# plainerman/DiffDock-Pocket

Measured on AMD Instinct MI355X. Metric: ligand poses/sec (40 samples x 20 steps) on 3dpf, higher is better.
Workload: dtype f32 (fc and G products: fp16 hi/lo split of both operands on v_mfma_f32_16x16x32_f16 - the row-stationary conv kernel - and v_mfma_f32_32x32x16_f16, fp32 accumulate; G between its two kernels as fp16 hi + continuation byte = 19 significant bits; the exact fp32 MFMA form is timed in other_workloads)

## Files before the change

diffdock_pocket_amd/_lib.py:

```python
from __future__ import annotations

import ctypes as C
import operator
import os

HERE = os.path.dirname(os.path.abspath(__file__))
LIB_PATH = os.environ.get("DDP_HIP_LIB", os.path.join(HERE, "libddp_hip.so"))

DDP_MAX_TASKS, DDP_MAX_BLOCKS, DDP_MAX_SEGS, DDP_MAX_NS, DDP_EDGE_TILE = 9, 4, 3, 64, 64
F_SCALAR_S0, F_DOT, F_SCALAR_S1, F_VEC_S0, F_CROSS = range(5)
FS = 68

DDP_MAX_GEMM_BATCH = 16
DDP_EVAL_MAX_ATOMS = 1024
DDP_GUIDANCE_MAX_TORSIONS = 1024
DDP_MINIMIZE_MAX_ATOMS, DDP_MINIMIZE_MAX_TORSIONS = 512, 4096
DDP_MINIMIZE_FLEX_MAX_MOVING, DDP_MINIMIZE_FLEX_MAX_BONDS, DDP_MINIMIZE_FLEX_MAX_STATE_BYTES = 256, 256, 47040
DDP_SCORE_GUIDANCE_FLEX_MAX_ATOMS, DDP_SCORE_GUIDANCE_FLEX_MAX_TORSIONS = DDP_MINIMIZE_MAX_ATOMS, DDP_GUIDANCE_MAX_TORSIONS
DDP_SCORE_GUIDANCE_FLEX_MAX_MOVING, DDP_SCORE_GUIDANCE_FLEX_MAX_BONDS = DDP_MINIMIZE_FLEX_MAX_MOVING, DDP_MINIMIZE_FLEX_MAX_BONDS
DDP_PAIRWISE_MAX_SAMPLES, DDP_CLUSTER_MAX_SAMPLES = 32768, 1024
EXPORTS = ["ddp_conv_messages", "ddp_conv_rows", "ddp_stage_a_gh", "ddp_stage_a_gh3", "ddp_segment_reduce", "ddp_edge_featurize", "ddp_edge_featurize_jobs", "ddp_torsion_sh", "ddp_stage_a", "ddp_stage_a_h2",
           "ddp_pose_update", "ddp_sidechain_update", "ddp_sde_update", "ddp_radius_count", "ddp_radius_fill", "ddp_knn", "ddp_group_by_key", "ddp_node_linear", "ddp_scan_jobs", "ddp_mark_jobs", "ddp_rowcopy_jobs", "ddp_select_jobs",
           "ddp_gather_rows", "ddp_clean_pair_maps", "ddp_flex_mark", "ddp_fallback_rowmap", "ddp_step_prologue", "ddp_trrot_head", "ddp_tor_head", "ddp_radius_search_jobs", "ddp_group_by_key_jobs", "ddp_set_occupancy_shaping", "ddp_pose_rmsd", "ddp_pose_contacts", "ddp_pose_pairwise_rmsd", "ddp_pose_cluster", "ddp_traj_record", "ddp_svgd_tau", "ddp_svgd_pairs", "ddp_svgd_rows", "ddp_refine_energy", "ddp_refine_direction", "ddp_refine_accept", "ddp_clash_guidance", "ddp_score_guidance", "ddp_score_guidance_flex", "ddp_pose_score", "ddp_pose_profile", "ddp_pose_minimize", "ddp_pose_minimize_flex", "ddp_pose_search", "ddp_pose_search_select", "ddp_pose_search_flex", "ddp_pocket_occupancy", "ddp_pocket_buriedness", "ddp_pocket_label", "ddp_conv_deal_tile", "ddp_abi_version", "ddp_last_error", "ddp_source_hash"]


class Seg(C.Structure):
    _fields_ = [("kind", C.c_int32), ("in_off", C.c_int32), ("count", C.c_int32)]


class Block(C.Structure):
    _fields_ = [("U", C.c_int32), ("n", C.c_int32), ("C", C.c_int32), ("out_off", C.c_int32), ("tile0", C.c_int32),
                ("ntiles", C.c_int32), ("nsub", C.c_int32), ("ups", C.c_int32), ("nseg", C.c_int32),
                ("seg", Seg * DDP_MAX_SEGS), ("g_slot", C.c_int32), ("g_col0", C.c_int32)]


class RoleSeg(C.Structure):
    _fields_ = [("block", C.c_int32), ("tile0", C.c_int32), ("tstride", C.c_int32), ("count", C.c_int32), ("round", C.c_int32)]


DDP_CONV32_WAVES, DDP_MAX_ROLE_SEGS = 4, 2


class ConvShape(C.Structure):
    _fields_ = [("f_in", C.c_int32), ("hid", C.c_int32), ("kp1", C.c_int32), ("hp", C.c_int32), ("hs", C.c_int32),
                ("nct1", C.c_int32), ("d_out", C.c_int32), ("nblocks", C.c_int32), ("fbuf_floats", C.c_int32),
                ("g_cols", C.c_int32 * 2), ("blk", Block * DDP_MAX_BLOCKS), ("nrounds", C.c_int32),
                ("nrole", C.c_int32 * DDP_CONV32_WAVES), ("role", (RoleSeg * DDP_MAX_ROLE_SEGS) * DDP_CONV32_WAVES)]


class ConvTask(C.Structure):
    _fields_ = [("x_src", C.c_void_p), ("ldx_src", C.c_int32), ("n_edges", C.c_int32), ("src", C.c_void_p),
                ("eid", C.c_void_p), ("sh", C.c_void_p), ("seg_ptr", C.c_void_p * DDP_MAX_SEGS),
                ("seg_idx", C.c_void_p * DDP_MAX_SEGS), ("seg_ld", C.c_int32 * DDP_MAX_SEGS),
                ("seg_n", C.c_int32 * DDP_MAX_SEGS), ("w1p", C.c_void_p), ("b1p", C.c_void_p), ("w2p", C.c_void_p),
                ("b2p", C.c_void_p), ("msg", C.c_void_p), ("g", C.c_void_p * 2),
                ("pos", C.c_void_p), ("n_edges_dev", C.c_void_p), ("w1h", C.c_void_p), ("w2h", C.c_void_p), ("h2_range_flag", C.c_void_p),
                ("wsh", C.c_void_p), ("bsp", C.c_void_p), ("gh", C.c_void_p * 2), ("gh_fmt", C.c_int32), ("rows_form", C.c_int32), ("rows_bias_k", C.c_int32), ("rows_seg0", C.c_int32), ("rows_seg1", C.c_int32), ("rows_nts", C.c_int32)]


class ReduceSrc(C.Structure):
    _fields_ = [("msg", C.c_void_p), ("rowptr", C.c_void_p), ("bn_scale", C.c_void_p), ("bn_shift", C.c_void_p),
                ("n_edges", C.c_int32), ("rowmap", C.c_void_p), ("n_edges_dev", C.c_void_p)]


DDP_MAX_NODE_JOBS, DDP_MAX_NODE_CAT = 8, 16
DDP_MAX_LIST_JOBS = 12
_P, _I = C.c_void_p, C.c_int32


class ScanJob(C.Structure):
    _fields_ = [("n", _I), ("n_dev", _P), ("flag", _P), ("val", _P), ("rowptr", _P), ("base", _I), ("excl", _P), ("excl2", _P),
                ("list", _P), ("total", _P)]


class MarkJob(C.Structure):
    _fields_ = [("idx", _P), ("n", _I), ("n_dev", _P), ("mask", _P)]


class RowcopyJob(C.Structure):
    _fields_ = [("n_rows", _I), ("keep", _P), ("old_rowptr", _P), ("new_rowptr", _P), ("inp", _P * 3), ("out", _P * 3)]


class SelectJob(C.Structure):
    _fields_ = [("n", _I), ("n_dev", _P), ("mask_a", _P), ("idx_a", _P), ("mask_b", _P), ("idx_b", _P), ("out_idx", _P),
                ("pay", _P * 4), ("pay_add", _I * 4), ("out", _P * 4), ("total", _P), ("block_count", _P), ("block_off", _P)]


class RadiusJob(C.Structure):
    _fields_ = [("x", _P), ("x_ptr", _P), ("y", _P), ("y_batch", _P), ("ny", _I), ("r", C.c_float), ("max_neighbors", _I),
                ("flags", _I), ("graph_div", _P), ("counts", _P), ("offsets", _P), ("base", _I), ("total", _P), ("out_query", _P),
                ("out_x", _P), ("capacity", _I), ("overflow", _P)]


class SdeArgs(C.Structure):
    _fields_ = [("score", _P * 4), ("z", _P * 4), ("out", _P * 4), ("n", _I * 4)]


class SvgdArgs(C.Structure):
    _fields_ = [("pos", _P), ("n", _I), ("n_lig", _I), ("n_tor", _I), ("dihedrals", _P), ("score", _P * 3), ("upd", _P * 3), ("gdt", _P),
                ("weight", C.c_float), ("w_rep", C.c_float), ("w_rot", C.c_float), ("w_tor", C.c_float), ("svgd_only", _I),
                ("tau", _P), ("tr_diff", _P), ("rot_diff", _P), ("tor_diff", _P), ("dist", _P)]


class RefineArgs(C.Structure):
    _fields_ = [("n_samples", _I), ("n", _I), ("m", _I), ("rec_stride", _I), ("n_tor", _I), ("pos", _P), ("anchor", _P), ("lig_radii", _P),
                ("rec", _P), ("rec_radii", _P), ("self_pairs", _P), ("overlap", C.c_double), ("restraint", C.c_double), ("energy", _P),
                ("grad", _P), ("bonds", _P), ("mask_rotate", _P), ("step", _P), ("tr", _P), ("rot", _P), ("tor", _P), ("trial", _P),
                ("trial_energy", _P), ("trial_grad", _P), ("accepted", _P), ("grow", C.c_double), ("shrink", C.c_double),
                ("step_max", C.c_double)]


class GuidanceArgs(C.Structure):
    _fields_ = [("n_samples", _I), ("n", _I), ("m", _I), ("rec_stride", _I), ("n_tor", _I), ("pos", _P), ("lig_radii", _P), ("rec", _P),
                ("rec_radii", _P), ("self_pairs", _P), ("bonds", _P), ("mask_rotate", _P), ("overlap", C.c_double), ("weight", _P),
                ("max_tr", C.c_double), ("max_rot", C.c_double), ("max_tor", C.c_double), ("upd", _P * 3), ("energy", _P), ("grad", _P)]


class ScoreForm(C.Structure):
    _fields_ = [(k, C.c_double) for k in ("cutoff", "gauss_offset", "gauss_width", "hydrophobic_good", "hydrophobic_bad", "hbond_good",
                                          "hbond_bad", "w_gauss", "w_repulsion", "w_hydrophobic", "w_hbond")]
    _read = operator.attrgetter(*(k for k, _ in _fields_))

    @classmethod
    def from_config(cls, config) -> "ScoreForm":
        return cls(*cls._read(config))


class ScoreArgs(C.Structure):
    _anonymous_ = ("form",)
    _fields_ = [("n_samples", _I), ("n", _I), ("m", _I), ("rec_stride", _I), ("pos", _P), ("lig_radii", _P), ("lig_flags", _P), ("rec", _P),
                ("rec_radii", _P), ("rec_flags", _P), ("self_pairs", _P), ("form", ScoreForm), ("tor_divisor", C.c_double), ("energy", _P),
                ("grad", _P)]


class ScoreGuidanceArgs(C.Structure):
    _anonymous_ = ("form",)
    _fields_ = [("n_samples", _I), ("n", _I), ("m", _I), ("rec_stride", _I), ("n_tor", _I), ("pos", _P), ("lig_radii", _P), ("lig_flags", _P),
                ("rec", _P), ("rec_radii", _P), ("rec_flags", _P), ("self_pairs", _P), ("bonds", _P), ("mask_rotate", _P), ("form", ScoreForm),
                ("weight", _P), ("max_tr", C.c_double), ("max_rot", C.c_double), ("max_tor", C.c_double), ("upd", _P * 3), ("energy", _P),
                ("grad", _P)]


class ScoreGuidanceFlexArgs(C.Structure):
    _anonymous_ = ("form",)
    _fields_ = ScoreGuidanceArgs._fields_[:-2] + [("n_mov", _I), ("n_sc", _I), ("n_sub", _I), ("reserved", _I), ("mov", _P), ("sc_edge_idx", _P),
                                                  ("sc_sub", _P), ("sc_map", _P), ("sc_pairs", _P), ("max_sc", C.c_double), ("upd_sc", _P),
                                                  ("energy", _P), ("grad_mov", _P)]


class ProfileArgs(C.Structure):
    _anonymous_ = ("form",)
    _fields_ = [("n_samples", _I), ("n", _I), ("m", _I), ("rec_stride", _I), ("n_res", _I), ("reserved", _I), ("pos", _P), ("lig_radii", _P),
                ("lig_flags", _P), ("rec", _P), ("rec_radii", _P), ("rec_flags", _P), ("res_ptr", _P), ("form", ScoreForm),
                ("contact_distance", C.c_double), ("profile", _P), ("bits", _P)]


class MinimizeArgs(C.Structure):
    _anonymous_ = ("form",)
    _fields_ = [("n_samples", _I), ("n", _I), ("m", _I), ("rec_stride", _I), ("n_tor", _I), ("iterations", _I), ("pos", _P), ("anchor", _P),
                ("lig_radii", _P), ("lig_flags", _P), ("rec", _P), ("rec_radii", _P), ("rec_flags", _P), ("self_pairs", _P), ("bonds", _P),
                ("mask_rotate", _P), ("form", ScoreForm), ("restraint", C.c_double), ("grow", C.c_double), ("shrink", C.c_double),
                ("step_max", C.c_double), ("step", _P), ("accepted", _P), ("energy_in", _P), ("energy_out", _P), ("history", _P), ("grad", _P)]


class MinimizeFlexArgs(C.Structure):
    _anonymous_ = ("form",)
    _fields_ = MinimizeArgs._fields_ + [("rec_anchor", _P), ("n_mov", _I), ("n_sc", _I), ("n_sub", _I), ("reserved", _I), ("mov", _P),
                                        ("sc_edge_idx", _P), ("sc_sub", _P), ("sc_map", _P), ("sc_pairs", _P),
                                        ("restraint_sc", C.c_double), ("grad_mov", _P)]


class SearchArgs(C.Structure):
    _fields_ = [("min", MinimizeArgs), ("replicas", _I), ("cycles", _I), ("cycle0", _I), ("reserved", _I), ("step_init", C.c_double),
                ("temperature", C.c_double), ("perturb", _P), ("u", _P), ("cur_pos", _P), ("cur_e", _P), ("best_pos", _P), ("best_e", _P),
                ("best_cycle", _P), ("accepted", _P), ("trace", _P), ("flags", _P), ("starts", _P)]


class SearchFlexArgs(C.Structure):
    _fields_ = [("flex", MinimizeFlexArgs), ("replicas", _I), ("cycles", _I), ("cycle0", _I), ("reserved", _I), ("step_init", C.c_double),
                ("temperature", C.c_double), ("perturb", _P), ("u", _P), ("cur_pos", _P), ("cur_mov", _P), ("cur_e", _P), ("best_pos", _P),
                ("best_mov", _P), ("best_e", _P), ("best_cycle", _P), ("accepted", _P), ("trace", _P), ("flags", _P), ("starts", _P),
                ("starts_mov", _P)]


class SearchSelectArgs(C.Structure):
    _fields_ = [("n_samples", _I), ("n", _I), ("replicas", _I), ("reserved", _I), ("best_pos", _P), ("best_e", _P), ("best_cycle", _P),
                ("pos_out", _P), ("energy_out", _P), ("replica_out", _P), ("cycle_out", _P)]


def flex_state_bytes(n: int, n_mov: int, n_sc: int) -> int:
    return 89 * n + 81 * n_mov + 4 * n_sc


class GroupJob(C.Structure):
    _fields_ = [("key", _P), ("n_items", _I), ("n_items_dev", _P), ("n_keys", _I), ("pay", _P * 3), ("rowptr", _P), ("perm", _P),
                ("out_key", _P), ("out", _P * 3), ("key_map", _P), ("scratch", _P)]



DDP_MAX_FEATURIZE_JOBS = 8


class FeaturizeJob(C.Structure):
    _fields_ = [("pos_a", _P), ("ia", _P), ("pos_b", _P), ("ib", _P), ("n_edges", _I), ("n_edges_dev", _P), ("offset", _P), ("k_rbf", _I),
                ("coeff", C.c_float), ("pre", _P), ("pre_idx", _P), ("ld_pre", _I), ("pre2", _P), ("n_pre2", _I), ("ld_pre2", _I),
                ("w1d", _P), ("w2", _P), ("b2", _P), ("ns", _I), ("out", _P), ("sh", _P)]


class _BondJob(C.Structure):
    _fields_ = [("pos", _P), ("b0", _P), ("b1", _P), ("n", _I), ("mid", _P), ("vec", _P)]


class _CopyJob(C.Structure):
    _fields_ = [("src", _P), ("dst", _P), ("n", _I)]


class PrologueArgs(C.Structure):
    _fields_ = [("t", _P * 4), ("t_stride", _I * 4), ("sig_min", C.c_float * 4), ("sig_max", C.c_float * 4), ("sigma", _P * 4),
                ("n_graphs", _I), ("cut", _P), ("cut_mul", C.c_float), ("cut_add", C.c_float), ("graph_emb", _P), ("sd", _I),
                ("emb_scale", C.c_float), ("freq", _P), ("lig_pos", _P), ("graph_ptr", _P), ("center", _P),
                ("bonds", _BondJob * 2), ("copy", _CopyJob * 2)]


class TrRotArgs(C.Structure):
    _fields_ = [("gp", _P), ("ld_gp", _I), ("n_graphs", _I), ("ns", _I), ("sd", _I), ("graph_emb", _P), ("w1", _P * 2), ("b1", _P * 2),
                ("w2", _P * 2), ("b2", _P * 2), ("sigma", _P * 2), ("so3_table", _P), ("so3_n", _I), ("so3_lo", C.c_float),
                ("so3_span", C.c_float), ("out", _P * 2)]


class TorArgs(C.Structure):
    _fields_ = [("h", _P), ("ld_h", _I), ("n_bonds", _I), ("ns", _I), ("w1", _P), ("w2", _P), ("sigma", _P), ("graph_of_bond", _P),
                ("torus_table", _P), ("torus_n", _I), ("torus_lo", C.c_float), ("torus_span", C.c_float), ("out", _P)]


class NodeJob(C.Structure):
    _fields_ = [("n_rows", C.c_int32), ("cat", C.c_void_p), ("ld_cat", C.c_int32), ("n_cat", C.c_int32), ("table", C.c_void_p),
                ("feat_off", C.c_int32 * DDP_MAX_NODE_CAT), ("emb_dim", C.c_int32), ("emb_mode", C.c_int32),
                ("dense", C.c_void_p * 2), ("ld_dense", C.c_int32 * 2), ("n_dense", C.c_int32 * 2),
                ("t", C.c_void_p), ("t_stride", C.c_int32), ("scale", C.c_float), ("freq", C.c_void_p),
                ("sig_emb", C.c_void_p), ("ld_sig", C.c_int32), ("sd", C.c_int32), ("sig_out", C.c_void_p), ("ld_sig_out", C.c_int32),
                ("w", C.c_void_p), ("bias", C.c_void_p),
                ("out", C.c_void_p), ("ld_out", C.c_int32), ("ncols", C.c_int32), ("zero_to", C.c_int32),
                ("add", C.c_void_p), ("ld_add", C.c_int32)]


def g_ld(hid: int, gcols: int) -> int:
    return (((hid + 3) // 4 * 4 + 1) * gcols + 31) // 32 * 32


class DdpError(RuntimeError):
    pass


_lib = None


def load():
    global _lib
    if _lib is not None:
        return _lib
    if not os.path.exists(LIB_PATH):
        raise DdpError(f"{LIB_PATH} not found: build it with `python -m diffdock_pocket_amd.build` "
                       f"(hipcc --offload-arch=gfx950); there is no fallback path")
    lib = C.CDLL(LIB_PATH)
    for name in EXPORTS:
        if not hasattr(lib, name):
            raise DdpError(f"{LIB_PATH} does not export {name}")
    lib.ddp_abi_version.restype = C.c_int
    lib.ddp_last_error.restype = C.c_char_p
    lib.ddp_conv_messages.argtypes = [C.POINTER(ConvShape), C.POINTER(ConvTask), C.c_int, C.c_void_p]
    lib.ddp_conv_messages.restype = C.c_int
    lib.ddp_conv_rows.argtypes = lib.ddp_conv_messages.argtypes
    lib.ddp_conv_rows.restype = C.c_int
    lib.ddp_segment_reduce.argtypes = [C.c_void_p, C.c_int, C.c_int, C.c_int, C.POINTER(ReduceSrc), C.c_int, C.c_int,
                                       C.c_int, C.c_int, C.c_void_p]
    lib.ddp_segment_reduce.restype = C.c_int
    lib.ddp_edge_featurize.argtypes = [C.c_void_p, C.c_void_p, C.c_void_p, C.c_void_p, C.c_int, C.c_void_p, C.c_void_p, C.c_int,
                                       C.c_float, C.c_void_p, C.c_void_p, C.c_int, C.c_void_p, C.c_int, C.c_int, C.c_void_p,
                                       C.c_void_p, C.c_void_p, C.c_int, C.c_void_p, C.c_void_p, C.c_void_p]
    lib.ddp_edge_featurize.restype = C.c_int
    lib.ddp_edge_featurize_jobs.argtypes = [C.POINTER(FeaturizeJob), C.c_int, C.c_void_p]
    lib.ddp_edge_featurize_jobs.restype = C.c_int
    lib.ddp_torsion_sh.argtypes = [C.c_void_p, C.c_void_p, C.c_void_p, C.c_int, C.c_void_p, C.c_void_p, C.c_void_p, C.c_int, C.c_int,
                                   C.c_void_p, C.c_void_p, C.c_int, C.c_void_p, C.c_void_p]
    lib.ddp_torsion_sh.restype = C.c_int
    lib.ddp_stage_a.argtypes = [C.c_void_p, C.c_int, C.c_int, C.c_void_p, C.c_void_p, C.c_int, C.POINTER(C.c_int32), C.c_int,
                                C.c_void_p, C.c_void_p, C.c_int, C.c_int, C.c_void_p, C.c_int, C.c_void_p]
    lib.ddp_stage_a.restype = C.c_int
    lib.ddp_stage_a_h2.argtypes = lib.ddp_stage_a.argtypes[:-1] + [C.c_void_p, C.c_void_p]
    lib.ddp_stage_a_h2.restype = C.c_int
    lib.ddp_stage_a_gh.argtypes = lib.ddp_stage_a_h2.argtypes[:-1] + [C.c_void_p, C.c_void_p]
    lib.ddp_stage_a_gh.restype = C.c_int
    lib.ddp_stage_a_gh3.argtypes = lib.ddp_stage_a_gh.argtypes
    lib.ddp_stage_a_gh3.restype = C.c_int
    lib.ddp_set_occupancy_shaping.argtypes = [C.c_int, C.c_int]
    lib.ddp_set_occupancy_shaping.restype = C.c_int
    lib.ddp_pose_update.argtypes = [C.c_void_p, C.c_int, C.c_int, C.c_void_p, C.c_void_p, C.c_void_p, C.c_int, C.c_void_p,
                                    C.c_void_p, C.c_void_p, C.c_void_p]
    lib.ddp_pose_update.restype = C.c_int
    lib.ddp_sidechain_update.argtypes = [C.c_void_p, C.c_int, C.c_int, C.c_void_p, C.c_int, C.c_void_p, C.c_void_p, C.c_void_p,
                                         C.c_void_p, C.c_void_p]
    lib.ddp_sidechain_update.restype = C.c_int
    lib.ddp_radius_count.argtypes = [C.c_void_p, C.c_void_p, C.c_void_p, C.c_void_p, C.c_int, C.c_float, C.c_int, C.c_int,
                                     C.c_void_p, C.c_void_p]
    lib.ddp_radius_count.restype = C.c_int
    lib.ddp_radius_fill.argtypes = [C.c_void_p, C.c_void_p, C.c_void_p, C.c_void_p, C.c_int, C.c_float, C.c_int, C.c_int,
                                    C.c_void_p, C.c_void_p, C.c_void_p, C.c_void_p]
    lib.ddp_radius_fill.restype = C.c_int
    lib.ddp_knn.argtypes = [C.c_void_p, C.c_void_p, C.c_void_p, C.c_int, C.c_int, C.c_void_p, C.c_void_p]
    lib.ddp_knn.restype = C.c_int
    lib.ddp_group_by_key.argtypes = [C.c_void_p, C.c_int, C.c_int] + [C.c_void_p] * 11
    lib.ddp_group_by_key.restype = C.c_int
    for name, job in (("ddp_scan_jobs", ScanJob), ("ddp_mark_jobs", MarkJob), ("ddp_rowcopy_jobs", RowcopyJob),
                      ("ddp_select_jobs", SelectJob), ("ddp_radius_search_jobs", RadiusJob), ("ddp_group_by_key_jobs", GroupJob)):
        getattr(lib, name).argtypes = [C.POINTER(job), C.c_int, C.c_void_p]
        getattr(lib, name).restype = C.c_int
    lib.ddp_sde_update.argtypes = [C.c_void_p, C.POINTER(SdeArgs), C.c_void_p]
    lib.ddp_sde_update.restype = C.c_int
    lib.ddp_gather_rows.argtypes = [C.c_void_p, C.c_int, C.c_void_p, C.c_int, C.c_void_p, C.c_void_p, C.c_int, C.c_int, C.c_void_p]
    lib.ddp_gather_rows.restype = C.c_int
    lib.ddp_clean_pair_maps.argtypes = [C.c_void_p, C.c_void_p, C.c_void_p, C.c_void_p, C.c_int, C.c_int, C.c_int, C.c_int, C.c_void_p,
                                        C.c_void_p, C.c_void_p]
    lib.ddp_clean_pair_maps.restype = C.c_int
    lib.ddp_flex_mark.argtypes = [C.c_void_p, C.c_void_p, C.c_int, C.c_void_p, C.c_void_p, C.c_int, C.c_int, C.c_int, C.c_int, C.c_int,
                                  C.c_void_p, C.c_void_p]
    lib.ddp_flex_mark.restype = C.c_int
    lib.ddp_fallback_rowmap.argtypes = [C.c_void_p, C.c_void_p, C.c_void_p, C.c_void_p, C.c_int, C.c_int, C.c_void_p, C.c_void_p]
    lib.ddp_fallback_rowmap.restype = C.c_int
    for name, st in (("ddp_step_prologue", PrologueArgs), ("ddp_trrot_head", TrRotArgs), ("ddp_tor_head", TorArgs)):
        getattr(lib, name).argtypes = [C.POINTER(st), C.c_void_p]
        getattr(lib, name).restype = C.c_int
    lib.ddp_node_linear.argtypes = [C.POINTER(NodeJob), C.c_int, C.c_void_p]
    lib.ddp_node_linear.restype = C.c_int
    lib.ddp_pose_rmsd.argtypes = [C.c_void_p, C.c_int, C.c_int, C.c_void_p, C.c_int, C.c_void_p, C.c_int, C.c_void_p, C.c_int,
                                  C.c_void_p, C.c_void_p, C.c_void_p]
    lib.ddp_pose_rmsd.restype = C.c_int
    lib.ddp_pose_contacts.argtypes = [C.c_void_p, C.c_int, C.c_int, C.c_void_p, C.c_void_p, C.c_int, C.c_int, C.c_void_p, C.c_float,
                                      C.c_void_p, C.c_void_p, C.c_void_p]
    lib.ddp_pose_contacts.restype = C.c_int
    lib.ddp_pose_pairwise_rmsd.argtypes = [C.c_void_p, C.c_int, C.c_int, C.c_void_p, C.c_int, C.c_void_p, C.c_int, C.c_void_p, C.c_void_p]
    lib.ddp_pose_pairwise_rmsd.restype = C.c_int
    lib.ddp_pose_cluster.argtypes = [C.c_void_p, C.c_int, C.c_void_p, C.c_float, C.c_void_p, C.c_void_p, C.c_void_p, C.c_void_p, C.c_void_p]
    lib.ddp_pose_cluster.restype = C.c_int
    lib.ddp_traj_record.argtypes = [C.c_void_p, C.c_int, C.c_int, C.c_void_p, C.c_void_p, C.c_int, C.c_void_p, C.c_int, C.c_void_p,
                                    C.c_int, C.c_void_p, C.c_void_p]
    lib.ddp_traj_record.restype = C.c_int
    for name in ("ddp_svgd_tau", "ddp_svgd_pairs", "ddp_svgd_rows"):
        getattr(lib, name).argtypes = [C.POINTER(SvgdArgs), C.c_void_p]
        getattr(lib, name).restype = C.c_int
    for name in ("ddp_refine_energy", "ddp_refine_direction", "ddp_refine_accept"):
        getattr(lib, name).argtypes = [C.POINTER(RefineArgs), C.c_void_p]
        getattr(lib, name).restype = C.c_int
    lib.ddp_clash_guidance.argtypes = [C.POINTER(GuidanceArgs), C.c_void_p]
    lib.ddp_clash_guidance.restype = C.c_int
    lib.ddp_score_guidance.argtypes = [C.POINTER(ScoreGuidanceArgs), C.c_void_p]
    lib.ddp_score_guidance.restype = C.c_int
    lib.ddp_score_guidance_flex.argtypes = [C.POINTER(ScoreGuidanceFlexArgs), C.c_void_p]
    lib.ddp_score_guidance_flex.restype = C.c_int
    lib.ddp_pose_score.argtypes = [C.POINTER(ScoreArgs), C.c_void_p]
    lib.ddp_pose_score.restype = C.c_int
    lib.ddp_pose_profile.argtypes = [C.POINTER(ProfileArgs), C.c_void_p]
    lib.ddp_pose_profile.restype = C.c_int
    lib.ddp_pose_minimize.argtypes = [C.POINTER(MinimizeArgs), C.c_void_p]
    lib.ddp_pose_minimize.restype = C.c_int
    lib.ddp_pose_minimize_flex.argtypes = [C.POINTER(MinimizeFlexArgs), C.c_void_p]
    lib.ddp_pose_minimize_flex.restype = C.c_int
    lib.ddp_pose_search.argtypes = [C.POINTER(SearchArgs), C.c_void_p]
    lib.ddp_pose_search.restype = C.c_int
    lib.ddp_pose_search_select.argtypes = [C.POINTER(SearchSelectArgs), C.c_void_p]
    lib.ddp_pose_search_select.restype = C.c_int
    lib.ddp_pose_search_flex.argtypes = [C.POINTER(SearchFlexArgs), C.c_void_p]
    lib.ddp_pose_search_flex.restype = C.c_int
    lib.ddp_pocket_occupancy.argtypes = [C.c_void_p, C.c_void_p, C.c_int, C.c_float, C.c_float, C.c_float, C.c_float, C.c_int, C.c_int, C.c_int,
                                         C.c_void_p, C.c_void_p]
    lib.ddp_pocket_occupancy.restype = C.c_int
    lib.ddp_pocket_buriedness.argtypes = [C.c_void_p, C.c_int, C.c_int, C.c_int, C.c_double, C.c_double, C.c_int, C.c_void_p, C.c_void_p,
                                          C.c_void_p]
    lib.ddp_pocket_buriedness.restype = C.c_int
    lib.ddp_pocket_label.argtypes = [C.c_void_p, C.c_int, C.c_int, C.c_int, C.c_void_p, C.c_void_p]
    lib.ddp_pocket_label.restype = C.c_int
    lib.ddp_conv_deal_tile.argtypes = [C.c_int, C.c_int, C.c_int]
    lib.ddp_conv_deal_tile.restype = C.c_int
    if lib.ddp_abi_version() != 17:
        raise DdpError("libddp_hip.so ABI version mismatch")
    lib.ddp_source_hash.restype = C.c_char_p
    if "DDP_HIP_LIB" not in os.environ:
        from .build import source_hash
        have, want = lib.ddp_source_hash().decode(), source_hash()
        if have != want:
            raise DdpError(f"{LIB_PATH} was built from other sources (library {have}, tree {want}): rebuild it with "
                           f"`python -m diffdock_pocket_amd.build`")
    _lib = lib
    return lib


def check(rc, what):
    if rc != 0:
        raise DdpError(f"{what} failed (rc={rc}): {load().ddp_last_error().decode()}")
```

diffdock_pocket_amd/csrc/ddp_conv_rows.hip:

```cpp
#include <hip/hip_runtime.h>
#include <stdint.h>
#include <stdio.h>
#include <stdlib.h>

#undef DDP_STAMPS
#include "ddp_conv_rows_common.h"

#ifndef DDP_ROWS_GRING1
#define DDP_ROWS_GRING1 12
#endif
#ifndef DDP_ROWS_GRING3
#define DDP_ROWS_GRING3 8
#endif

#ifdef DDP_ROWS_STAMPS
#define RS_SLOTS 32
#define RS_WGS 16384
__device__ unsigned long long ddp_rows_stamp_buf[(size_t)RS_WGS * ROWS_NW * RS_SLOTS];
#define RSTAMP(k)                                                                                          \
  do {                                                                                                     \
    unsigned long long t_;                                                                                 \
    __builtin_amdgcn_sched_barrier(0);                                                                     \
    asm volatile("s_memtime %0\n\ts_waitcnt lgkmcnt(0)" : "=s"(t_)::"memory");                          \
    __builtin_amdgcn_sched_barrier(0);                                                                     \
// ... 486 lines not shown
  {
    int lo = 1 << 30, hi = 0;
    for (int bi = 0; bi < S.nblocks; ++bi)
      if (S.blk[bi].ntiles > 0)
        for (int si = 0; si < S.blk[bi].nseg; ++si) {
          lo = min(lo, S.blk[bi].seg[si].in_off);
          hi = max(hi, S.blk[bi].seg[si].in_off + 3 * S.blk[bi].seg[si].count);
        }
    const float* __restrict__ xs = T.x_src + (size_t)src * T.ldx_src;
#pragma unroll
    for (int i = 0; i < 2; ++i) vtouch[i] = (hi > lo) ? xs[min(lo + 32 * (2 * i + hh), hi - 1)] : 0.f;
  }

  rows_request_piece<NS>(ring, wsh, 0, ROWS_NP * RL.nts, 0, wave, lane);
  rows_request_piece<NS>(ring, wsh, 1, ROWS_NP * RL.nts, 1, wave, lane);
  for (int i = tid; i < RL.nts * 32; i += ROWS_NT) lbias[i] = T.bsp[i];
  RSTAMP(1);
  h8 xh[NS];
  f32x4* xlo = reinterpret_cast<f32x4*>(priv);
  {
    f32x4 xv[NS][2];
#pragma unroll
    for (int ks = 0; ks < NS; ++ks)
#pragma unroll
      for (int q = 0; q < 2; ++q) {
        const int kq = 4 * ks + 2 * hh + q;
        const int sg = kq / NQ, off = kq - sg * NQ;
        const float* __restrict__ b = (sg == 0) ? xb0 : (sg == 1) ? xb1 : xb2;
        xv[ks][q] = (sg < 3) ? reinterpret_cast<const f32x4*>(b)[off] : f32x4{0.f, 0.f, 0.f, 0.f};
      }
#pragma unroll
    for (int ks = 0; ks < NS; ++ks) {
      h4 h0, l0, h1, l1;
      rows_split(xv[ks][0], ROWS_SX, h0, l0, T.h2_range_flag);
      rows_split(xv[ks][1], ROWS_SX, h1, l1, T.h2_range_flag);
      h8 lo;
#pragma unroll
      for (int i = 0; i < 4; ++i) {
        xh[ks][i] = h0[i];
        xh[ks][4 + i] = h1[i];
        lo[i] = l0[i];
        lo[4 + i] = l1[i];
      }
      xlo[ks * 64 + lane] = __builtin_bit_cast(f32x4, lo);
    }
  }

  RSTAMP(2);
  asm volatile("" ::"v"(vtouch[0]), "v"(vtouch[1]));
  h8 ah[NS], al[NS];
  int t = 0;
#pragma unroll
  for (int ct = 0; ct < NCT1; ++ct, ++t) {
    f32x16 acc;
#pragma unroll
    for (int pc = 0; pc < ROWS_NP; ++pc) {
      constexpr int KPP = NS / ROWS_NP, PIECE_Q = 2 * KPP * 64;
      if (pc == 0) rows_stream_step<NS, 0>(ring, wsh, t, RL.nts, wave, lane);
      else if (pc == 1) rows_stream_step<NS, 1>(ring, wsh, t, RL.nts, wave, lane);
      else rows_stream_step<NS, 2>(ring, wsh, t, RL.nts, wave, lane);
      if (pc == 0) {
        const f32x4* bp = reinterpret_cast<const f32x4*>(lbias + t * 32 + 4 * hh);
#pragma unroll
        for (int q4 = 0; q4 < 4; ++q4) {
          const f32x4 b = bp[2 * q4];
#pragma unroll
          for (int q = 0; q < 4; ++q) acc[4 * q4 + q] = b[q];
        }
      }
      const f32x4* slot = ring + pc * PIECE_Q;
      f32x4 w0 = slot[lane], w1 = slot[64 + lane];
      f32x4 xl = xlo[(pc * KPP) * 64 + lane];
#pragma unroll
      for (int k = 0; k < KPP; ++k) {
        const int ks = pc * KPP + k;
        const h8 wh = __builtin_bit_cast(h8, w0), wl = __builtin_bit_cast(h8, w1), xlk = __builtin_bit_cast(h8, xl);
        if (k + 1 < KPP) {
          w0 = slot[(2 * k + 2) * 64 + lane];
          w1 = slot[(2 * k + 3) * 64 + lane];
          xl = xlo[(ks + 1) * 64 + lane];
        }
        acc = __builtin_amdgcn_mfma_f32_32x32x16_f16(wh, xh[ks], acc, 0, 0, 0);
        acc = __builtin_amdgcn_mfma_f32_32x32x16_f16(wh, xlk, acc, 0, 0, 0);
        acc = __builtin_amdgcn_mfma_f32_32x32x16_f16(wl, xh[ks], acc, 0, 0, 0);
      }
    }
#pragma unroll
    for (int j = 0; j < 16; ++j) {
      const float pre = acc[j] * (ROWS_SH / (ROWS_SW * ROWS_SX));
      h2_range_check(pre, T.h2_range_flag);
      const float v = fmaxf(pre, 0.f);
      const _Float16 hi = (_Float16)v;
      const _Float16 lo = (_Float16)(v - (float)hi);
      if (2 * ct + (j >> 3) < NS) {
        ah[2 * ct + (j >> 3)][j & 7] = hi;
        al[2 * ct + (j >> 3)][j & 7] = lo;
      }
    }
  }

  RSTAMP(3);
  float* F = reinterpret_cast<float*>(priv);
  RowsAux* aux = reinterpret_cast<RowsAux*>(priv + RL.aux_off);
  unsigned rmask;
  {
    const int prev = __shfl_up(src, 1);
    const bool rowv = (hh == 0) && (r < nvw);
    const bool runstart = rowv && (r == 0 || src != prev);
    rmask = (unsigned)(__ballot(runstart) & 0xffffffffull);
    const unsigned upto = (r == 31) ? ~0u : ((2u << r) - 1u);
    if (hh == 0) {
      aux->src[r] = src;
      aux->pos[r] = pos;
      aux->rid[r] = rowv ? (int)__popc(rmask & upto) - 1 : -1;
      constexpr float fs = 1.f / (ROWS_SH * ROWS_SW), gs = 1.f / (ROWS_SH * ROWS_SG);
      aux->sh[r][0] = shv[0] * fs; aux->sh[r][1] = shv[1] * fs; aux->sh[r][2] = shv[2] * fs; aux->sh[r][3] = shv[3] * fs;
      aux->shT[0][r] = shv[0] * gs; aux->shT[1][r] = shv[1] * gs; aux->shT[2][r] = shv[2] * gs; aux->shT[3][r] = shv[3] * gs;
    }
  }

  RSTAMP(4);
  RSTAMP_VAL(30, __popc(rmask));
  RSTAMP_VAL(31, p0 / ROWS_ET);
  int sgi = 0;
  for (int bi = 0; bi < S.nblocks; ++bi) {
    const ddp_block_t& B = S.blk[bi];
    if (B.ntiles > 0 && B.U > 0) {
      bool fast = true;
      for (int si = 0; si < B.nseg; ++si)
        fast = fast && B.seg[si].count <= 16 && (B.seg[si].kind == DDP_F_DOT || B.seg[si].kind == DDP_F_VEC_S0 || B.seg[si].kind == DDP_F_CROSS);
      if (fast)
        rows_build_features<8>(B, T, aux, F, lane);
      else
        build_features<32, 2>(B, T, aux->src, aux->sh, F, lane);
    }
    const int nparts = (B.n + 31) >> 5;
    for (int part = 0; part < nparts; ++part, ++sgi) {
      int gmode = 0;
      if (B.C == 3 && B.g_slot >= 0 && nparts == 1 && 2 * B.n <= 32) {
        const bool with_next = bi + 1 < S.nblocks && S.blk[bi + 1].C == 3 && S.blk[bi + 1].g_slot >= 0 && S.blk[bi + 1].n == B.n;
        const bool with_prev = bi > 0 && S.blk[bi - 1].C == 3 && S.blk[bi - 1].g_slot >= 0 && S.blk[bi - 1].n == B.n;
        const bool prev_is_second = with_prev && bi > 1 && S.blk[bi - 2].C == 3 && S.blk[bi - 2].g_slot >= 0 && S.blk[bi - 2].n == B.n;
        if (with_prev && !prev_is_second) gmode = 2;
        else if (with_next) gmode = 1;
      }
      if (B.C == 1)
        t = rows_segment<NS, 1, G3>(RL, B, bi, part, T, ah, al, ring, lbias, t, F, aux, rmask, src, nvw, wave, lane, sgi, 0);
      else
        t = rows_segment<NS, 3, G3>(RL, B, bi, part, T, ah, al, ring, lbias, t, F, aux, rmask, src, nvw, wave, lane, sgi, gmode);
    }
  }
}

int ddp_conv_rows_plan(const ddp_conv_shape_t* shape, const ddp_conv_task_t* tasks, int ntasks, RowsPlan* plan) {
  if (!shape || !tasks) return ddp_fail(DDP_EINVAL, "ddp_conv_rows: null argument");
  if (ntasks < 0 || ntasks > DDP_MAX_TASKS) return ddp_fail(DDP_ELIMIT, "ddp_conv_rows: ntasks > DDP_MAX_TASKS");
  if (shape->nblocks < 1 || shape->nblocks > DDP_MAX_BLOCKS) return ddp_fail(DDP_EINVAL, "ddp_conv_rows: nblocks");
  const int sc = (shape->f_in != shape->hid) ? 0 : (shape->hid == 180) ? 60 : (shape->hid == 96) ? 32 : 0;
  if (sc == 0) return ddp_fail(DDP_EINVAL, "ddp_conv_rows: shapes of the size classes ns = 60 / 32 (f_in = hid = 180 / 96) only");
  RowsPlan& P = *plan;
  ConvLaunch& L = P.L;
  L.shape = *shape;
  L.r1_floats = 0;
  L.tv_off = 0;
  L.ntasks = 0;
  L.dev_counts = 0;
  L.deal_c = ddp_conv_deal_chunk();
  const int NS = (sc == 60) ? 12 : 6, nct1 = shape->nct1;
  if (nct1 != (shape->hid + 31) / 32) return ddp_fail(DDP_EINVAL, "ddp_conv_rows: nct1");
  int nts = nct1, frows = 0;
  for (int b = 0; b < shape->nblocks; ++b) {
    const ddp_block_t& B = shape->blk[b];
    if (B.C != 1 && B.C != 3) return ddp_fail(DDP_EINVAL, "ddp_conv_rows: block C must be 1 or 3");
    if (B.n < 1 || B.n > 64 || (B.C == 3 && B.n > 32)) return ddp_fail(DDP_ELIMIT, "ddp_conv_rows: block n too large");
    if (B.nsub < 1 || B.nsub > 2 || B.ups < 1 || (B.nsub > 1) != (B.n > 32) || (B.nsub == 1 && B.ups != 32 / B.n))
      return ddp_fail(DDP_EINVAL, "ddp_conv_rows: nsub / ups");
    if (B.g_slot > 1 || (B.g_slot >= 0 && (shape->g_cols[B.g_slot] < B.g_col0 + B.n)))
      return ddp_fail(DDP_EINVAL, "ddp_conv_rows: factorised block outside its G row");
    if (B.out_off < 0 || B.out_off + B.n * B.C > shape->d_out) return ddp_fail(DDP_EINVAL, "ddp_conv_rows: block outside the message row");
    if (B.nseg < 0 || B.nseg > DDP_MAX_SEGS) return ddp_fail(DDP_EINVAL, "ddp_conv_rows: nseg");
    if (B.ntiles > 0 && B.U > 0) {
      nts += ((B.n + 31) / 32) * (B.nsub > 1 ? B.U : (B.U + B.ups - 1) / B.ups);
      if (B.U * B.C > frows) frows = B.U * B.C;
    }
  }
  int tiles = 0, gfmt = -1, form = -1, bias_k = -1;
  for (int i = 0; i < ntasks; ++i) {
    const ddp_conv_task_t& T = tasks[i];
    if (T.n_edges <= 0) continue;
    if (T.gh_fmt != 0 && T.gh_fmt != 1) return ddp_fail(DDP_EINVAL, "ddp_conv_rows: task.gh_fmt must be 0 or 1");
    if (gfmt >= 0 && T.gh_fmt != gfmt) return ddp_fail(DDP_EINVAL, "ddp_conv_rows: the tasks of a launch carry G in ONE plane form");
    gfmt = T.gh_fmt;
    if (T.rows_form != 0 && T.rows_form != 1) return ddp_fail(DDP_EINVAL, "ddp_conv_rows: task.rows_form must be 0 or 1");
    if ((T.rows_bias_k != 0 || T.rows_seg0 != 0 || T.rows_seg1 != 0 || T.rows_nts != 0) && T.rows_form != 1)
      return ddp_fail(DDP_EINVAL, "ddp_conv_rows: task.rows_bias_k / rows_seg0 / rows_seg1 / rows_nts need rows_form 1");
    if (form >= 0 && T.rows_form != form) return ddp_fail(DDP_EINVAL, "ddp_conv_rows: the tasks of a launch carry ONE form of operand images");
    form = T.rows_form;
    if (T.rows_seg0 < 0 || T.rows_seg1 < 0 || T.rows_nts < 0 || (T.rows_seg1 > 0 && (T.rows_seg1 <= T.rows_seg0 || T.rows_nts < nct1)) ||
        (T.rows_nts > nts) || (T.rows_seg1 > 0 && !T.rows_bias_k))
      return ddp_fail(DDP_EINVAL, "ddp_conv_rows: task.rows_seg0 / rows_seg1 / rows_nts");
    if ((bias_k >= 0 && T.rows_bias_k != bias_k) || (unsigned)T.rows_bias_k > 1u || (T.rows_bias_k && (shape->hid & 15) == 0))
      return ddp_fail(DDP_EINVAL, "ddp_conv_rows: rows_bias_k is 0 or 1 for all tasks of a launch and needs hid % 16 != 0");
    bias_k = T.rows_bias_k;
    if (T.n_edges_dev) L.dev_counts = 1;
    if (!T.wsh || !T.bsp || (reinterpret_cast<size_t>(T.wsh) & 15) || (reinterpret_cast<size_t>(T.bsp) & 15))
      return ddp_fail(DDP_EINVAL, "ddp_conv_rows: task.wsh / bsp missing (or not 16-byte aligned)");
    for (int gs = 0; gs < 2; ++gs)
      if (shape->g_cols[gs] > 0 && (!T.gh[gs] || (reinterpret_cast<size_t>(T.gh[gs]) & 15)))
        return ddp_fail(DDP_EINVAL, "ddp_conv_rows: factorised shape but task.gh is null (or not 16-byte aligned)");
    for (int sg = 0; sg < 3; ++sg)
      if (T.seg_n[sg] != shape->f_in / 3 || (T.seg_ld[sg] & 3) || (reinterpret_cast<size_t>(T.seg_ptr[sg]) & 15) || !T.seg_idx[sg])
        return ddp_fail(DDP_EINVAL, "ddp_conv_rows: edge_attr_ must be three 16-byte aligned segments of f_in / 3 columns");
    if (reinterpret_cast<size_t>(T.sh) & 15) return ddp_fail(DDP_EINVAL, "ddp_conv_rows: sh must be 16-byte aligned");
    L.tile_start[L.ntasks] = tiles;
    L.task[L.ntasks] = T;
    tiles += (T.n_edges + ROWS_ET - 1) / ROWS_ET;
    ++L.ntasks;
  }
  L.tile_start[L.ntasks] = tiles;
  P.sc = sc;
  P.form = form;
  P.gh_fmt = gfmt;
  P.tiles = tiles;
  if (tiles == 0) return 0;
  P.nts = nts;
  if (form == 1 && frows > R16_FROWS) frows = R16_FROWS;
  P.frows = frows;
  int fbytes = frows * ROWS_FS * 4;
  fbytes = (fbytes + 127) / 128 * 128;
  P.aux_off = fbytes;
  int priv = fbytes + (int)sizeof(RowsAux);
  if (form == 0) priv += 2048;
  if (priv < NS * 1024) priv = NS * 1024;
  priv = (priv + 127) / 128 * 128;
  P.priv_bytes = priv;
  P.bias_tiles = (form == 1 && bias_k) ? nct1 : nts;
  P.bias_bytes = (P.bias_tiles * 128 + 127) / 128 * 128;
  size_t lds_bytes = (size_t)2 * (NS * 1024) + P.bias_bytes + (size_t)ROWS_NW * priv;
  if (2 * lds_bytes > 160 * 1024) return ddp_fail(DDP_ELIMIT, "ddp_conv_rows: LDS budget of two workgroups per CU exceeded (too many vector features per block)");
  if ((size_t)ddp_shape_rows_min_lds > lds_bytes) lds_bytes = (size_t)ddp_shape_rows_min_lds;
  P.lds_bytes = lds_bytes;
  return 0;
}

extern "C" int ddp_conv_rows(const ddp_conv_shape_t* shape, const ddp_conv_task_t* tasks, int ntasks, void* stream) {
  RowsPlan P;
  const int rc = ddp_conv_rows_plan(shape, tasks, ntasks, &P);
  if (rc != 0 || P.tiles == 0) return rc;
  if (P.form == 1) return ddp_conv_rows16_launch(P, stream);
  RowsLaunch RL;
  RL.L = P.L;
  RL.nts = P.nts;
  RL.bias_bytes = P.bias_bytes;
  RL.priv_bytes = P.priv_bytes;
  RL.aux_off = P.aux_off;
  static int lds_have[4] = {0, 0, 0, 0};
  hipError_t err;
  if (P.sc == 60) {
    if (P.gh_fmt == 1) ROWS_LAUNCH((ddp_conv_rows_kernel<60, 1>), 2, "hipFuncSetAttribute(conv rows)")
    else ROWS_LAUNCH((ddp_conv_rows_kernel<60, 0>), 0, "hipFuncSetAttribute(conv rows)")
  } else {
    if (P.gh_fmt == 1) ROWS_LAUNCH((ddp_conv_rows_kernel<32, 1>), 3, "hipFuncSetAttribute(conv rows)")
    else ROWS_LAUNCH((ddp_conv_rows_kernel<32, 0>), 1, "hipFuncSetAttribute(conv rows)")
  }
  err = hipGetLastError();
  if (err != hipSuccess) return ddp_fail_hip(err, "ddp_conv_rows launch");
  return 0;
}
```

diffdock_pocket_amd/csrc/ddp_conv_rows16.hip:

```cpp
#include <hip/hip_runtime.h>
#include <stdint.h>
#include <stdio.h>
#include <stdlib.h>

#undef DDP_STAMPS
#include "ddp_conv_rows_common.h"

typedef int i32x4 __attribute__((ext_vector_type(4)));

#ifdef DDP_DEAL_STAMPS
#define DS_WGS 16384
__device__ unsigned long long ddp_deal_stamp_buf[(size_t)DS_WGS * 8];
__device__ __forceinline__ unsigned long long ddp_deal_now() {
  unsigned long long t;
  __builtin_amdgcn_sched_barrier(0);
  asm volatile("s_memrealtime %0\n\ts_waitcnt lgkmcnt(0)" : "=s"(t)::"memory");
  __builtin_amdgcn_sched_barrier(0);
  return t;
}
#define DSTAMP_BEGIN(task_, tile_)                                                                     \
  do {                                                                                                 \
    const unsigned long long t_ = ddp_deal_now();                                                      \
    unsigned xcc_;                                                                                     \
    asm volatile("s_getreg_b32 %0, hwreg(HW_REG_XCC_ID)" : "=s"(xcc_));                                \
// ... 281 lines not shown
#pragma unroll
  for (int ct = 0; ct < 2; ++ct) {
    const int c = 16 * ct + n;
    if (B.nsub > 1) {
      ncol[ct] = 32 * part + c;
      us[ct] = 0;
      valid[ct] = ncol[ct] < B.n;
    } else {
      us[ct] = c / B.n;
      ncol[ct] = c - us[ct] * B.n;
      valid[ct] = us[ct] < B.ups;
    }
  }
  f32x16 res[C];
#pragma unroll
  for (int c = 0; c < C; ++c) res[c] = splat16(0.f);

  if constexpr (!DIRECT) {
    if (B.g_slot >= 0 && rmask != 0u) {
      const RowsGPart PA = rows_gpart_of<GF>(S, T, bi, part);
      if (PA.nmine > 16)
        r16_g_runs<NS, C, 2, GF>(S, PA, ah, al, aux, rmask, src_reg, lane, res);
      else
        r16_g_runs<NS, C, 1, GF>(S, PA, ah, al, aux, rmask, src_reg, lane, res);
    }
  }

  const int cnt = (B.ntiles == 0 || B.U == 0) ? 0 : (B.nsub > 1 ? B.U : (B.U + B.ups - 1) / B.ups);
  const int upt = (B.nsub > 1) ? 1 : B.ups;
  const bool chunked = B.U * C > RL.frows;
  const int tpc = chunked ? max(1, RL.frows / (C * upt)) : cnt;
  int u0 = 0;
  for (int j = 0; j < cnt; ++j, ++t) {
    constexpr int KPP = NS / ROWS_NP, PIECE_Q = 2 * KPP * 64;
    if (chunked && j % tpc == 0) {
      u0 = j * upt;
      r16_build_features_range(B, T, aux, F, lane, u0, min(B.U, u0 + tpc * upt));
    }
    f32x4 acc[4];
    rows_stream_step<NS, 0>(ring, wsh, t, nts, wave, lane);
    {
      const bool bt = t < RL.bias_tiles;
      const float b0 = bt ? lbias[t * 32 + n] : 0.f, b1 = bt ? lbias[t * 32 + 16 + n] : 0.f;
      acc[0] = r16_splat4(b0);
      acc[1] = r16_splat4(b1);
      acc[2] = r16_splat4(b0);
      acc[3] = r16_splat4(b1);
    }
    r16_piece<NS, 0>(ring, ah, al, lane, acc);
    rows_stream_step<NS, 1>(ring, wsh, t, nts, wave, lane);
    r16_piece<NS, 1>(ring + PIECE_Q, ah, al, lane, acc);
    rows_stream_step<NS, 2>(ring, wsh, t, nts, wave, lane);
    r16_piece<NS, 2>(ring + 2 * PIECE_Q, ah, al, lane, acc);
#pragma unroll
    for (int ct = 0; ct < 2; ++ct) {
      int u = (B.nsub > 1) ? j : j * B.ups + us[ct];
      if (!(valid[ct] && u < B.U)) u = 0;
      const float* frow = F + ((u - u0) * C) * ROWS_FS + 4 * g;
#pragma unroll
      for (int rt = 0; rt < 2; ++rt)
#pragma unroll
        for (int c = 0; c < C; ++c) {
          const f32x4 f = *reinterpret_cast<const f32x4*>(frow + c * ROWS_FS + 16 * rt);
#pragma unroll
          for (int q = 0; q < 4; ++q) res[c][4 * (2 * rt + ct) + q] += f[q] * acc[2 * rt + ct][q];
        }
    }
  }

  if (B.nsub == 1 && B.ups > 1 && cnt > 0) {
    for (int s = 1; s < B.ups; ++s) {
      const int csrc = min(n + s * B.n, 31);
      const int from = (csrc & 15) + 16 * g;
      const bool hi_tile = csrc >= 16;
#pragma unroll
      for (int c = 0; c < C; ++c)
#pragma unroll
        for (int rt = 0; rt < 2; ++rt)
#pragma unroll
          for (int q = 0; q < 4; ++q) {
            const float v0 = __shfl(res[c][4 * (2 * rt) + q], from), v1 = __shfl(res[c][4 * (2 * rt + 1) + q], from);
            if (us[0] == 0) res[c][4 * (2 * rt) + q] += hi_tile ? v1 : v0;
          }
    }
  }

  float* __restrict__ mo = T.msg + B.out_off;
#pragma unroll
  for (int ct = 0; ct < 2; ++ct) {
    if (valid[ct] && us[ct] == 0) {
#pragma unroll
      for (int rt = 0; rt < 2; ++rt) {
        const i32x4 pq = *reinterpret_cast<const i32x4*>(&aux->pos[16 * rt + 4 * g]);
#pragma unroll
        for (int q = 0; q < 4; ++q)
          if (16 * rt + 4 * g + q < nvw) {
#pragma unroll
            for (int c = 0; c < C; ++c) mo[(size_t)pq[q] * S.d_out + ncol[ct] * C + c] = res[c][4 * (2 * rt + ct) + q];
          }
      }
    }
  }
  return t;
}

template <int SZ, int GF, bool DIRECT>
__device__ __forceinline__ void r16_body(const R16Launch& RL) {
  constexpr int NS = H2Class<SZ>::NS, NS2 = NS / 2, RING_Q = 2 * NS * 64;
  constexpr int NQ = SZ / 4;
  static_assert(NS > 0 && NS % (2 * ROWS_NP) == 0 && SZ % 4 == 0, "size classes whose k16 steps split into ROWS_NP pieces of whole k32 steps");
  extern __shared__ __attribute__((aligned(16))) float lds[];
  const ConvLaunch& L = RL.L;
  const ddp_conv_shape_t& S = L.shape;
  const int tid = threadIdx.x;
  int ti, p0, nvalid;
  if (!conv_tile<ROWS_ET>(L, ti, p0, nvalid)) return;
  DSTAMP_BEGIN(ti, p0 / ROWS_ET);
  const ddp_conv_task_t& T = L.task[ti];
  const int wave = __builtin_amdgcn_readfirstlane(tid >> 6), lane = tid & 63, r = lane & 31, n = lane & 15, g = lane >> 4;
  f32x4* ring = reinterpret_cast<f32x4*>(lds);
  float* lbias = lds + RING_Q * 4;
  char* priv = reinterpret_cast<char*>(lds) + RING_Q * 16 + RL.bias_bytes + (size_t)wave * RL.priv_bytes;
  const int nts = (T.rows_nts > 0) ? T.rows_nts : RL.nts;
  const RowsStream wsh = rows_stream_of(T.wsh, nts, 2 * NS * 1024);
  const int nvw = max(0, min(32, nvalid - 32 * wave));

  const int pr = p0 + min(32 * wave + r, nvalid - 1);
  const int src = T.src[pr], eid = T.eid[pr];
  const int pos = T.pos ? T.pos[pr] : pr;
  const f32x4 shv = reinterpret_cast<const f32x4*>(T.sh)[eid];
  const float* __restrict__ xb[2][3];
#pragma unroll
  for (int et = 0; et < 2; ++et) {
    const int pe = p0 + min(32 * wave + 16 * et + n, nvalid - 1);
#pragma unroll
    for (int sg = 0; sg < 3; ++sg) xb[et][sg] = T.seg_ptr[sg] + (size_t)T.seg_idx[sg][pe] * T.seg_ld[sg];
  }
  float vtouch[2];
  {
    int lo = 1 << 30, hi = 0;
    for (int bi = 0; bi < S.nblocks; ++bi)
      if (S.blk[bi].ntiles > 0)
        for (int si = 0; si < S.blk[bi].nseg; ++si) {
          lo = min(lo, S.blk[bi].seg[si].in_off);
          hi = max(hi, S.blk[bi].seg[si].in_off + 3 * S.blk[bi].seg[si].count);
        }
    const float* __restrict__ xs = T.x_src + (size_t)src * T.ldx_src;
#pragma unroll
    for (int i = 0; i < 2; ++i) vtouch[i] = (hi > lo) ? xs[min(lo + 32 * (2 * i + (lane >> 5)), hi - 1)] : 0.f;
  }

  rows_request_piece<NS>(ring, wsh, 0, ROWS_NP * nts, 0, wave, lane);
  rows_request_piece<NS>(ring, wsh, 1, ROWS_NP * nts, 1, wave, lane);
  for (int i = tid; i < RL.bias_tiles * 32; i += ROWS_NT) lbias[i] = T.bsp[i];
  h8 xh[NS];
  f32x4* xlo = reinterpret_cast<f32x4*>(priv);
  {
#pragma unroll
    for (int s = 0; s < NS2; ++s) {
      f32x4 xv[2][2];
#pragma unroll
      for (int et = 0; et < 2; ++et)
#pragma unroll
        for (int q = 0; q < 2; ++q) {
          const int kq = 8 * s + 2 * g + q;
          const int sg = kq / NQ, off = kq - sg * NQ;
          const float* __restrict__ b = (sg == 0) ? xb[et][0] : (sg == 1) ? xb[et][1] : xb[et][2];
          xv[et][q] = (sg < 3) ? reinterpret_cast<const f32x4*>(b)[off] : f32x4{0.f, 0.f, 0.f, 0.f};
        }
#pragma unroll
      for (int et = 0; et < 2; ++et) {
        h4 h0, l0, h1, l1;
        rows_split(xv[et][0], ROWS_SX, h0, l0, T.h2_range_flag);
        rows_split(xv[et][1], ROWS_SX, h1, l1, T.h2_range_flag);
        h8 lo;
#pragma unroll
        for (int i = 0; i < 4; ++i) {
          xh[2 * s + et][i] = h0[i];
          xh[2 * s + et][4 + i] = h1[i];
          lo[i] = l0[i];
          lo[4 + i] = l1[i];
        }
        xlo[(2 * s + et) * 64 + lane] = __builtin_bit_cast(f32x4, lo);
      }
    }
  }
  asm volatile("" ::"v"(vtouch[0]), "v"(vtouch[1]));

  h8 ah[NS], al[NS];
  int t = 0;
#pragma unroll
  for (int ct = 0; ct < NS2; ++ct, ++t) {
    f32x4 acc[4];
#pragma unroll
    for (int pc = 0; pc < ROWS_NP; ++pc) {
      constexpr int KPP = NS / ROWS_NP, KP2 = KPP / 2, PIECE_Q = 2 * KPP * 64;
      if (pc == 0) rows_stream_step<NS, 0>(ring, wsh, t, nts, wave, lane);
      else if (pc == 1) rows_stream_step<NS, 1>(ring, wsh, t, nts, wave, lane);
      else rows_stream_step<NS, 2>(ring, wsh, t, nts, wave, lane);
      if (pc == 0) {
#pragma unroll
        for (int mt = 0; mt < 2; ++mt) {
          const f32x4 b = *reinterpret_cast<const f32x4*>(lbias + t * 32 + 16 * mt + 4 * g);
          acc[2 * mt] = b;
          acc[2 * mt + 1] = b;
        }
      }
      const f32x4* slot = ring + pc * PIECE_Q;
#pragma unroll
      for (int k = 0; k < KP2; ++k) {
        const int s = pc * KP2 + k;
        h8 w[2][2];
#pragma unroll
        for (int mt = 0; mt < 2; ++mt)
#pragma unroll
          for (int pl = 0; pl < 2; ++pl) w[mt][pl] = __builtin_bit_cast(h8, slot[((2 * k + mt) * 2 + pl) * 64 + lane]);
#pragma unroll
        for (int et = 0; et < 2; ++et) {
          const h8 xl = __builtin_bit_cast(h8, xlo[(2 * s + et) * 64 + lane]);
#pragma unroll
          for (int mt = 0; mt < 2; ++mt) {
            f32x4 d = acc[2 * mt + et];
            d = __builtin_amdgcn_mfma_f32_16x16x32_f16(w[mt][0], xh[2 * s + et], d, 0, 0, 0);
            d = __builtin_amdgcn_mfma_f32_16x16x32_f16(w[mt][0], xl, d, 0, 0, 0);
            d = __builtin_amdgcn_mfma_f32_16x16x32_f16(w[mt][1], xh[2 * s + et], d, 0, 0, 0);
            acc[2 * mt + et] = d;
          }
        }
      }
    }
#pragma unroll
    for (int et = 0; et < 2; ++et)
#pragma unroll
      for (int i = 0; i < 8; ++i) {
        const float pre = acc[2 * (i >> 2) + et][i & 3] * (ROWS_SH / (ROWS_SW * ROWS_SX));
        h2_range_check(pre, T.h2_range_flag);
        const float v = fmaxf(pre, 0.f);
        const _Float16 hi = (_Float16)v;
        ah[2 * ct + et][i] = hi;
        al[2 * ct + et][i] = (_Float16)(v - (float)hi);
      }
  }

  float* F = reinterpret_cast<float*>(priv);
  RowsAux* aux = reinterpret_cast<RowsAux*>(priv + RL.aux_off);
  unsigned rmask;
  {
    const int prev = __shfl_up(src, 1);
    const bool rowv = (lane < 32) && (r < nvw);
    const bool runstart = rowv && (r == 0 || src != prev);
    rmask = (unsigned)(__ballot(runstart) & 0xffffffffull);
    const unsigned upto = (r == 31) ? ~0u : ((2u << r) - 1u);
    if (lane < 32) {
      aux->src[r] = src;
      aux->pos[r] = pos;
      aux->rid[r] = rowv ? (int)__popc(rmask & upto) - 1 : -1;
      constexpr float fs = 1.f / (ROWS_SH * ROWS_SW), gs = 1.f / (ROWS_SH * ROWS_SG);
      aux->sh[r][0] = shv[0] * fs; aux->sh[r][1] = shv[1] * fs; aux->sh[r][2] = shv[2] * fs; aux->sh[r][3] = shv[3] * fs;
      aux->shT[0][r] = shv[0] * gs; aux->shT[1][r] = shv[1] * gs; aux->shT[2][r] = shv[2] * gs; aux->shT[3][r] = shv[3] * gs;
    }
  }

  const int seg0 = T.rows_seg0, seg1 = (T.rows_seg1 > 0) ? T.rows_seg1 : 0x7fffffff;
  int sgi = 0;
  for (int bi = 0; bi < S.nblocks; ++bi) {
    const ddp_block_t& B = S.blk[bi];
    const int nparts = (B.n + 31) >> 5;
    if (sgi >= seg1 || sgi + nparts <= seg0) {
      sgi += nparts;
      continue;
    }
    if (B.ntiles > 0 && B.U > 0 && B.U * B.C <= RL.frows) {
      bool fast = true;
      for (int si = 0; si < B.nseg; ++si)
        fast = fast && B.seg[si].count <= 16 && (B.seg[si].kind == DDP_F_DOT || B.seg[si].kind == DDP_F_VEC_S0 || B.seg[si].kind == DDP_F_CROSS);
      if (fast)
        rows_build_features<8>(B, T, aux, F, lane);
      else
        build_features<32, 2>(B, T, aux->src, aux->sh, F, lane);
    }
    for (int part = 0; part < nparts; ++part, ++sgi) {
      if (sgi < seg0 || sgi >= seg1) continue;
      if (B.C == 1)
        t = r16_segment<NS, 1, GF, DIRECT>(RL, B, bi, part, T, ah, al, ring, lbias, t, F, aux, rmask, src, nvw, wave, lane, nts);
      else
        t = r16_segment<NS, 3, GF, DIRECT>(RL, B, bi, part, T, ah, al, ring, lbias, t, F, aux, rmask, src, nvw, wave, lane, nts);
    }
  }
  DSTAMP_END();
}

template <int SZ, int GF>
__global__ __launch_bounds__(ROWS_NT, 2) void ddp_conv_rows16_kernel(const R16Launch RL) {
  r16_body<SZ, GF, false>(RL);
}
template <int SZ>
__global__ __launch_bounds__(ROWS_NT, 2) void ddp_conv_rows16_direct_kernel(const R16Launch RL) {
  r16_body<SZ, 0, true>(RL);
}

int ddp_conv_rows16_launch(const RowsPlan& P, void* stream) {
  R16Launch RL;
  RL.L = P.L;
  RL.nts = P.nts;
  RL.bias_tiles = P.bias_tiles;
  RL.bias_bytes = P.bias_bytes;
  RL.priv_bytes = P.priv_bytes;
  RL.aux_off = P.aux_off;
  RL.frows = P.frows;
  static int lds_have[6] = {0, 0, 0, 0, 0, 0};
  hipError_t err;
  const bool direct = P.L.shape.g_cols[0] == 0 && P.L.shape.g_cols[1] == 0;
  if (direct) {
    if (P.sc == 60) ROWS_LAUNCH((ddp_conv_rows16_direct_kernel<60>), 4, "hipFuncSetAttribute(conv rows16)")
    else ROWS_LAUNCH((ddp_conv_rows16_direct_kernel<32>), 5, "hipFuncSetAttribute(conv rows16)")
  } else if (P.sc == 60) {
    if (P.gh_fmt == 1) ROWS_LAUNCH((ddp_conv_rows16_kernel<60, 1>), 2, "hipFuncSetAttribute(conv rows16)")
    else ROWS_LAUNCH((ddp_conv_rows16_kernel<60, 0>), 0, "hipFuncSetAttribute(conv rows16)")
  } else {
    if (P.gh_fmt == 1) ROWS_LAUNCH((ddp_conv_rows16_kernel<32, 1>), 3, "hipFuncSetAttribute(conv rows16)")
    else ROWS_LAUNCH((ddp_conv_rows16_kernel<32, 0>), 1, "hipFuncSetAttribute(conv rows16)")
  }
  err = hipGetLastError();
  if (err != hipSuccess) return ddp_fail_hip(err, "ddp_conv_rows (16x16x32 form) launch");
  return 0;
}
```

diffdock_pocket_amd/csrc/ddp_conv_rows_common.h:

```cpp
#ifndef DDP_CONV_ROWS_COMMON_H
#define DDP_CONV_ROWS_COMMON_H
#include "ddp_conv_common.h"

#define ROWS_NW 4
#define ROWS_NT 256
#define ROWS_ET 128
#define ROWS_FS 36
#define ROWS_NP 3
#define R16_FROWS 72

#define ROWS_SX ((float)DDP_ROWS_SX)
#define ROWS_SW ((float)DDP_ROWS_SW)
#define ROWS_SH ((float)DDP_ROWS_SH)
#define ROWS_SG ((float)DDP_ROWS_SG)
__device__ __forceinline__ void rows_split(const f32x4 v, float scale, h4& hi, h4& lo, int32_t* flag) {
#pragma unroll
  for (int i = 0; i < 4; ++i) {
    const float V = v[i] * scale;
    h2_range_check(V, flag);
    hi[i] = (_Float16)V;
    lo[i] = (_Float16)(V - (float)hi[i]);
  }
}

struct RowsLaunch {
  ConvLaunch L;
  int nts;
  int bias_bytes;
  int priv_bytes;
  int aux_off;
};
struct R16Launch {
  ConvLaunch L;
  int nts;
  int bias_tiles;
  int bias_bytes;
  int priv_bytes;
  int aux_off;
  int frows;
};
static_assert(sizeof(ConvLaunch) + 16 <= 4096, "the launch descriptor travels as a kernel argument");

struct RowsAux {
  float shT[4][32];
  float sh[32][4];
  int src[32], pos[32], rid[32];
};

typedef __attribute__((address_space(3))) void* rows_lds_ptr_t;
typedef __amdgpu_buffer_rsrc_t RowsStream;
__device__ __forceinline__ RowsStream rows_stream_of(const void* wsh, int nts, int tile_bytes) {
  return __builtin_amdgcn_make_buffer_rsrc(const_cast<void*>(wsh), 0, nts * tile_bytes, 0x00020000);
}
template <int NS>
__device__ __forceinline__ void rows_request_piece(f32x4* ring, RowsStream wsh, int jn, int npieces, int slot, int wave, int lane) {
  constexpr int FPP = 2 * NS / ROWS_NP, FPW = FPP / ROWS_NW, PIECE_Q = FPP * 64;
  static_assert(NS % ROWS_NP == 0 && FPP % ROWS_NW == 0, "every wave moves the same number of fragments per piece");
  f32x4* nslot = ring + slot * PIECE_Q;
  const int piece_off = min(jn, npieces - 1) * (PIECE_Q * 16);
#pragma unroll
  for (int f = 0; f < FPW; ++f)
    __builtin_amdgcn_raw_ptr_buffer_load_lds(wsh, (rows_lds_ptr_t)(nslot + (wave + ROWS_NW * f) * 64), 16, ((wave + ROWS_NW * f) * 64 + lane) * 16, piece_off, 0, 0);
}
template <int NS, int P>
__device__ __forceinline__ void rows_stream_step(f32x4* ring, RowsStream wsh, int t, int nts, int wave, int lane) {
  constexpr int FPW = 2 * NS / ROWS_NP / ROWS_NW;
  static_assert(FPW == 2 || FPW == 1, "the literals below");
  if constexpr (FPW == 2)
    asm volatile("s_waitcnt vmcnt(2)" ::: "memory");
  else
    asm volatile("s_waitcnt vmcnt(1)" ::: "memory");
  asm volatile("s_waitcnt lgkmcnt(0)" ::: "memory");
  __builtin_amdgcn_s_barrier();
  asm volatile("" ::: "memory");
  rows_request_piece<NS>(ring, wsh, ROWS_NP * t + P + 2, ROWS_NP * nts, (P + 2) % ROWS_NP, wave, lane);
}

template <int MAXI>
__device__ __forceinline__ void rows_build_features(const ddp_block_t& B, const ddp_conv_task_t& T, const RowsAux* aux, float* F, int lane) {
  constexpr int FS = ROWS_FS;
  const int e = lane & 31, half = lane >> 5;
  const float* __restrict__ xrow = T.x_src + (size_t)aux->src[e] * T.ldx_src;
  const float s0 = aux->sh[e][0], sx = aux->sh[e][1], sy = aux->sh[e][2], sz = aux->sh[e][3];
  const float inv_sqrt3 = 0.57735026918962576f, inv_sqrt2 = 0.70710678118654752f;
  int ubase = 0;
  for (int si = 0; si < B.nseg; ++si) {
    const int kind = B.seg[si].kind, off = B.seg[si].in_off, cnt = B.seg[si].count;
    float ax[MAXI], ay[MAXI], az[MAXI];
#pragma unroll
    for (int i = 0; i < MAXI; ++i) {
      const int ul = max(min(half + 2 * i, cnt - 1), 0);
      ax[i] = xrow[off + 3 * ul];
      ay[i] = xrow[off + 3 * ul + 1];
      az[i] = xrow[off + 3 * ul + 2];
    }
#pragma unroll
    for (int i = 0; i < MAXI; ++i) {
      const int ul = half + 2 * i;
      if (ul < cnt) {
        const int u = ubase + ul;
        if (kind == DDP_F_DOT) {
          F[u * FS + e] = (ax[i] * sx + ay[i] * sy + az[i] * sz) * inv_sqrt3;
        } else if (kind == DDP_F_VEC_S0) {
          F[(u * 3 + 0) * FS + e] = ax[i] * s0;
          F[(u * 3 + 1) * FS + e] = ay[i] * s0;
          F[(u * 3 + 2) * FS + e] = az[i] * s0;
        } else {
          F[(u * 3 + 0) * FS + e] = (ay[i] * sz - az[i] * sy) * inv_sqrt2;
          F[(u * 3 + 1) * FS + e] = (az[i] * sx - ax[i] * sz) * inv_sqrt2;
          F[(u * 3 + 2) * FS + e] = (ax[i] * sy - ay[i] * sx) * inv_sqrt2;
        }
      }
    }
    ubase += cnt;
  }
}

struct RowsGPart {
  const char* base;
  size_t gldb;
  int wp, nmine, bias_off;
  int cumw;
};
#define ROWS_GPART_FILL(GF_, P_, S_, T_, B_, part_, wp_, cumw_, gcp_)                                            \
  {                                                                                                              \
    const int n8 = ((S_).hid + 7) >> 3;                                                                          \
    if constexpr ((GF_) == 1) {                                                                                  \
      (P_).base = reinterpret_cast<const char*>((T_).gh[(B_).g_slot]) + (size_t)(n8 * (cumw_)) * 24;             \
      (P_).gldb = (size_t)DDP_GH3_LD((S_).hid, (gcp_)) * 4;                                                      \
      (P_).bias_off = n8 * ((gcp_) - (cumw_)) * 24;                                                              \
    } else {                                                                                                     \
      (P_).base = reinterpret_cast<const char*>((T_).gh[(B_).g_slot]) + (size_t)(2 * n8 * (cumw_)) * 16;         \
      (P_).gldb = (size_t)DDP_GH_LD((S_).hid, (gcp_)) * 4;                                                       \
      (P_).bias_off = (8 * n8 * (gcp_) + (cumw_)) * 4 - (2 * n8 * (cumw_)) * 16;                                 \
    }                                                                                                            \
    (P_).wp = (wp_);                                                                                             \
    (P_).nmine = min(32, (B_).n - 32 * (part_));                                                                 \
    (P_).cumw = (cumw_);                                                                                         \
  }
template <int GF>
__device__ __forceinline__ RowsGPart rows_gpart_of(const ddp_conv_shape_t& S, const ddp_conv_task_t& T, int bi, int part) {
  const ddp_block_t& B = S.blk[bi];
  int wp = 0, cumw = 0, gcp = 0;
  for (int bj = 0; bj < S.nblocks; ++bj) {
    const ddp_block_t& Bj = S.blk[bj];
    if (Bj.g_slot != B.g_slot) continue;
    for (int pj = 0; pj < ((Bj.n + 31) >> 5); ++pj) {
      const int wj = (min(32, Bj.n - 32 * pj) + 3) & ~3;
      if (bj < bi || (bj == bi && pj < part)) cumw += wj;
      if (bj == bi && pj == part) wp = wj;
      gcp += wj;
    }
  }
  RowsGPart P;
  ROWS_GPART_FILL(GF, P, S, T, B, part, wp, cumw, gcp)
  return P;
}

struct RowsPlan {
  ConvLaunch L;
  int sc;
  int form, gh_fmt;
  int tiles;
  int nts;
  int bias_tiles;
  int bias_bytes, priv_bytes, aux_off;
  int frows;
  size_t lds_bytes;
};
int ddp_conv_rows_plan(const ddp_conv_shape_t* shape, const ddp_conv_task_t* tasks, int ntasks, RowsPlan* plan);
int ddp_conv_rows16_launch(const RowsPlan& P, void* stream);

#define ROWS_LAUNCH(KERNEL_, SLOT_, WHERE_)                                                                          \
  {                                                                                                                  \
    err = ddp_need_lds(reinterpret_cast<const void*>(KERNEL_), (int)P.lds_bytes, &lds_have[SLOT_]);                  \
    if (err != hipSuccess) return ddp_fail_hip(err, WHERE_);                                                         \
    hipLaunchKernelGGL(KERNEL_, dim3(P.tiles), dim3(ROWS_NT), P.lds_bytes, (hipStream_t)stream, RL);                 \
  }

#endif
```

diffdock_pocket_amd/engine.py:

```python
from __future__ import annotations

import ctypes as C
from collections.abc import Mapping
from types import SimpleNamespace
from typing import Dict, List, Optional

import math

import torch

from . import _lib as L
from . import graph as G
from . import launch as K
from . import packing as P
from . import packing as P_
from .graph import EdgeView

SRC_TYPE = {0: "l", 1: "r", 2: "a", 3: "a", 4: "l", 5: "r", 6: "r", 7: "l", 8: "a"}
RECV_TYPE = {0: "l", 1: "l", 2: "l", 3: "a", 4: "a", 5: "a", 6: "r", 7: "r", 8: "r"}
RECV_OF = {"a": (3, 4, 5), "r": (6, 7, 8)}
ORDER = {"l": [0, 2, 1], "a": [3, 4, 5], "r": [6, 8, 7]}
_DROP_SELF = 1


# ... 640 lines not shown
        if st is None or st.W.device != x.device:
            st = m._stage_a_stacks[key] = K.stage_a_stack([(k, conv.packed_g(x.device)) for k, conv in convs], convs[0][1].spec_g.hid, path)
        h2 = m.stage_a_h2 and K.CONV_H2 and not m.stage_a_bf16x3
        st.prepare(m.stage_a_h2, m.stage_a_bf16x3)
        Gall = torch.empty((len(st.meta), n_rows, st.ld), device=x.device, dtype=torch.float32)
        prof = K.profiler(hbm=True)
        if prof is not None:
            e0, e1 = torch.cuda.Event(enable_timing=True), torch.cuda.Event(enable_timing=True)
            e0.record()
        n_list = n_rows if rows is None else int(rows.shape[0])
        K.stage_a(x, n_list, st, Gall, rows=rows, rows_cnt=rows_cnt, out_rows=n_rows, h2=h2, x3=m.stage_a_bf16x3)
        if prof is not None:
            e1.record()
            row_bytes = 4.0 * len(st.meta) * (st.ld + st.W.shape[1])

            def nbytes(n_list=n_list, rows_cnt=rows_cnt, row_bytes=row_bytes, wn=st.W.numel()):
                n = n_list if rows_cnt is None else min(n_list, int(rows_cnt.item()))
                return row_bytes * n + 4.0 * wn
            prof.hbm.setdefault("ddp_stage_a_h2_kernel" if (st.path.rows or h2) else "ddp_stage_a_mfma_kernel", []).append((e0, e1, nbytes))
        return {(k, slot): Gall[i] for i, (k, slot, _) in enumerate(st.meta)}

    def _layers(self, S, F, dev, mark):
        m = self.m
        ns, L_, B, ldx = m.ns, m.num_conv_layers, S.B, m._ldx
        Nl, Nr, Na = S.Nl, S.Nr, S.Na
        c, so = F.c, F.so
        xl, xr, xa = F.xl, F.xr, F.xa
        e, sh = F.e, F.sh
        arr = {0: (xl, xl, "ll"), 1: (xl, xr, "lr"), 2: (xl, xa, "la"), 3: (xa, xa, "aa"), 4: (xa, xl, "la"), 5: (xa, xr, "ar"),
               6: (xr, xr, "rr"), 7: (xr, xl, "lr"), 8: (xr, xa, "ar")}
        nodes = {"l": (xl, Nl), "a": (xa, Na), "r": (xr, Nr)}
        dbg = m.debug_conv_outputs
        exact = getattr(F, "exact", None)
        prof_on = K.profiler() is not None
        plain = m.before_layers is not None
        fork = self._fork(dev) if (m.concurrent_small_batches and Na <= m.concurrent_max_atoms and not plain) else None
        pipelined = (fork is None and m.overlap_direct_conv and not plain and dbg is None and m.section_timer is None and L_ >= 2
                     and F.fact == {0, 1, 2, 3, 4, 5, 6, 7})
        side = self._fork(dev) if pipelined else None
        lists_fork = getattr(F, "lists_fork", None)

        def join_lists():
            nonlocal lists_fork
            if lists_fork is not None:
                lists_fork.join(only=4)
                lists_fork = None
        if not pipelined and fork is None:
            join_lists()

        def plan(l):
            P = SimpleNamespace(l=l, spec=m._layer_specs[l], spec_g=m._layer_specs_g[l], gmap={}, keep=[], msgs={})
            do_atom = m.flexible_sidechains or l != L_ - 1
            P.active = active = {"l": True, "a": do_atom, "r": do_atom and l != L_ - 1}
            P.shared = shared = F.shared0 if l == 0 else {}
            pl, pl_so = F.pruned.get(l, {}), F.pruned_so.get(l, {})
            P.c1 = c1 = F.clean1 if (l == 1 and F.clean1 is not None and active["a"]) else None
            P.per, P.groups = per, groups = {}, {}
            for k in range(9):
                rt, st_ = RECV_TYPE[k], SRC_TYPE[k]
                if not active[rt]:
                    continue
                csr, so_k = c[k], so.get(k) if k in F.fact else None
                x_src = arr[k][1]
                rows = ("all", None, None, nodes[st_][1])
                if k in pl:
                    csr, so_k = pl[k], pl_so.get(k)
                    if st_ != "l":
                        r_, rc = F.rows_a[l][st_]
                        rows = (f"pr{l}", r_, rc, nodes[st_][1])
                elif k in shared:
                    n0, e0, ns0 = shared[k]
                    csr = csr.prefix(e0, n0)
                    so_k = so_k.prefix(e0) if so_k is not None else None
                    x_src = x_src[:ns0]
                    rows = ("g0", None, None, ns0)
                elif k == 2 and so_k is not None:
                    rows = ("near", F.near_rows, F.cnt["near"], Na)
                    if exact is not None:
                        rows = ("near", F.near_rows[:exact[F.cnt["near"].data_ptr()]], None, Na)
                elif l in F.pruned and st_ != "l" and so_k is not None:
                    r_, rc = F.rows_a[l][st_]
                    rows = (f"pr{l}", r_, rc, nodes[st_][1])
                if exact is not None and rows[2] is not None:
                    rows = (rows[0], rows[1][:exact[rows[2].data_ptr()]], None, rows[3])
                per[k] = (csr, so_k, x_src)
                if so_k is not None and csr.n_edges > 0 and not (k == 3 and c1 is not None):
                    groups.setdefault((st_, rows[0]), (x_src, rows, []))[2].append((k, m.conv_layers[9 * l + k]))
            return P

        def node_bytes(l, k):
            d_in = P_.irreps_dim(P_.irreps_muls(ns, m.nv, l))
            return 4.0 * (nodes[SRC_TYPE[k]][1] * d_in + nodes[RECV_TYPE[k]][1] * m._layer_specs[l].d_out)

        def stage_a(P, which, forked=None):
            l = P.l
            for gi, ((st_, gid), (x_src, rows, convs)) in enumerate(P.groups.items()):
                if st_ not in which:
                    continue
                if forked is not None and gi > 0:
                    P.gmap.update(forked.run((gi - 1) % 3, lambda: self._stage_a(l, convs, x_src, rows[3], rows=rows[1], rows_cnt=rows[2])))
                else:
                    P.gmap.update(self._stage_a(l, convs, x_src, rows[3], rows=rows[1], rows_cnt=rows[2]))
            if forked is not None:
                for i_ in range(3):
                    forked.join(only=i_)
            c1 = P.c1
            if c1 is not None and "a" in which:
                conv3 = m.conv_layers[9 * l + 3]
                rows_d, rows_dc = c1.rows_d, c1.rows_d_cnt
                if exact is not None:
                    rows_d, rows_dc = rows_d[:exact[rows_dc.data_ptr()]], None
                P.g_d = self._stage_a(l, [(3, conv3)], xa, Na, rows=rows_d, rows_cnt=rows_dc)
                P.x_clean = torch.empty((c1.n0, ldx), device=dev)
                K.gather_rows(xa, c1.rows_v, c1.n0, P.x_clean, ldx)
                P.g_v = self._stage_a(l, [(3, conv3)], P.x_clean, c1.n0)
                P.keep += [P.g_d, P.g_v, P.x_clean]

        def direct_tasks(P):
            l, spec = P.l, P.spec
            direct = [(k, csr, x_src) for k, (csr, so_k, x_src) in P.per.items() if not (so_k is not None or (k == 3 and P.c1 is not None))]
            live = [(k, csr, x_src) for k, csr, x_src in direct if csr.n_edges > 0]
            split_cap = max(1, L.DDP_MAX_TASKS // max(1, len(live)))
            packs = direct_packs([(m.conv_layers[9 * l + k], max(1, min(m.direct_rows_max_split, split_cap, -(-256 // max(1, -(-csr.n_edges // 128))))))
                                  for k, csr, _ in live], dev)
            tasks, nb_d = [], 0.0
            for k, csr, x_src in direct:
                P.msgs[k] = (torch.empty((csr.n_edges, spec.d_out), device=dev), csr, m.conv_layers[9 * l + k].packed(dev))
            for (k, csr, x_src), pks in zip(live, packs):
                x_recv, _, ek = arr[k]
                if prof_on:
                    nb_d += node_bytes(l, k)
                segs = [(e[ek], csr.eid, ns, ns), (x_recv, csr.recv, ldx, ns), (x_src, csr.src, ldx, ns)]
                for i_, pk in enumerate(pks):
                    t_ = K.make_task(pk, K.conv_path(pk), x_src, ldx, csr, sh[ek], segs, P.msgs[k][0])
                    if i_:
                        t_._count = (0, None)
                    tasks.append(t_)
            P.tasks, P.nb_d = tasks, nb_d
            return tasks

        def launch_direct(P):
            K.launch_convs(P.spec, P.tasks, node_bytes=P.nb_d, tag=f"layer{P.l}")

        def launch_factorised(P, which="lar"):
            l, spec, c1 = P.l, P.spec, P.c1
            tasks_g, nb_g = [], 0.0
            for k, (csr, so_k, x_src) in P.per.items():
                if k in P.msgs or SRC_TYPE[k] not in which:
                    continue
                x_recv, _, ek = arr[k]
                conv = m.conv_layers[9 * l + k]
                pkc = conv.packed(dev)
                e_base, sh_k = e[ek], sh[ek]
                if k == 3 and c1 is not None:
                    msg = torch.empty((c1.E + c1.e0, spec.d_out), device=dev)
                    P.msgs[k] = (msg, csr, pkc, c1.rowmap)
                    pkg, path = conv.packed_g(dev), self._conv_path(conv, dev)
                    sd_ = c1.so_d
                    if sd_.n_edges > 0:
                        segs = [(e_base, sd_.eid, ns, ns), (x_recv, sd_.recv, ldx, ns), (xa, sd_.src, ldx, ns)]
                        tasks_g.append(K.make_task(pkg, path, xa, ldx, sd_, sh_k, segs, msg, g=[P.g_d.get((3, s_)) for s_ in (0, 1)]))
                    sv = c1.so_v
                    segs = [(e_base, sv.eid, ns, ns), (P.x_clean, sv.recv, ldx, ns), (P.x_clean, sv.src, ldx, ns)]
                    tasks_g.append(K.make_task(pkg, path, P.x_clean, ldx, sv, sh_k, segs, msg, g=[P.g_v.get((3, s_)) for s_ in (0, 1)]))
                    continue
                msg = torch.empty((csr.n_edges, spec.d_out), device=dev)
                P.msgs[k] = (msg, csr, pkc)
                if csr.n_edges == 0:
                    continue
                if prof_on:
                    nb_g += node_bytes(l, k)
                segs = [(e_base, so_k.eid, ns, ns), (x_recv, so_k.recv, ldx, ns), (x_src, so_k.src, ldx, ns)]
                tasks_g.append(K.make_task(conv.packed_g(dev), self._conv_path(conv, dev), x_src, ldx, so_k, sh_k, segs, msg,
                                           g=[P.gmap.get((k, s_)) for s_ in (0, 1)]))
            P.tasks_g = getattr(P, "tasks_g", []) + tasks_g
            if tasks_g:
                K.launch_convs(P.spec_g, tasks_g, flops_spec=spec, node_bytes=nb_g, tag=f"layer{l}")

        def fix_rowmaps(P):
            if P.l == 0 and F.flex0 is not None:
                for k, rm in F.flex0.rowmaps.items():
                    if k in P.msgs:
                        P.msgs[k] = (P.msgs[k][0], c[k], P.msgs[k][2], rm)

        def means(P, types):
            spec, shared = P.spec, P.shared
            for rt in types:
                if not P.active[rt]:
                    continue
                x, n = nodes[rt]
                own = [P.msgs[k] for k in ORDER[rt] if k not in shared]
                if own:
                    K.launch_reduce(x, ldx, n, spec.d_out, own, accumulate=True)
                com = [P.msgs[k] for k in ORDER[rt] if k in shared]
                if com:
                    n0 = shared[[k for k in ORDER[rt] if k in shared][0]][0]
                    K.launch_reduce(x, ldx, n0, spec.d_out, com, accumulate=True, n_rep=B, rep_stride=n0)

        if pipelined:
            P = plan(0)
            direct_tasks(P)
            if P.tasks:
                side.run(1, lambda P=P: launch_direct(P))
            stage_a(P, "lar")
            def atom_g_bytes(Pn):
                tot = 0
                for (st_, _gid), (_x, rows_, convs_) in (Pn.groups.items() if m.rows_all_or_none(dev) else ()):
                    if st_ != "a":
                        continue
                    for _k, conv_ in convs_:
                        tot += rows_[3] * 4 * sum(ld_ for ld_ in (conv_.packed_g(dev).gh_ld or []) if ld_ is not None)
                return tot
            for l in range(L_):
                nxt = plan(l + 1) if l + 1 < L_ else None
                launch_factorised(P)
                join_lists()
                fix_rowmaps(P)
                side.join(only=1)
                side.join(only=0)
                ev_r, ev_l, ev_sr, ev_sl = (torch.cuda.Event() for _ in range(4))

                def rec_chain(P=P, nxt=nxt, ev_r=ev_r, ev_sr=ev_sr):
                    means(P, "r")
                    ev_r.record()
                    if nxt is not None:
                        stage_a(nxt, "r")
                        ev_sr.record()

                def lig_chain(P=P, nxt=nxt, ev_l=ev_l, ev_sl=ev_sl):
                    means(P, "l")
                    ev_l.record()
                    if nxt is not None:
                        stage_a(nxt, "l")
                        ev_sl.record()
                side.run(3, rec_chain)
                side.run(2, lig_chain)
                means(P, "a")
                if nxt is not None:
                    direct_tasks(nxt)
                    if nxt.tasks:
                        def direct_next(nxt=nxt, ev_r=ev_r):
                            torch.cuda.current_stream(dev).wait_event(ev_r)
                            launch_direct(nxt)
                        side.run(1, direct_next)
                    if bool(getattr(m, "split_rows_launch", False)) and atom_g_bytes(nxt) >= m.split_rows_min_g_bytes:
                        def early(nxt=nxt, evs=(ev_r, ev_l, ev_sr, ev_sl)):
                            st_ = torch.cuda.current_stream(dev)
                            for ev in evs:
                                st_.wait_event(ev)
                            if getattr(m, "shape_early_rows", False):
                                K.occupancy_shaping(82 * 1024, 0)
                                try:
                                    launch_factorised(nxt, "rl")
                                finally:
                                    K.occupancy_shaping(0, 0)
                                return
                            launch_factorised(nxt, "rl")
                        side.run(0, early)
                    stage_a(nxt, "a")
                side.join(only=2)
                side.join(only=3)
                F.keep.append((P.keep, P.per, P.msgs, P.tasks, P.tasks_g, P.gmap, ev_r))
                P = nxt
            side.join()
            mark("reduce")
            return

        for l in range(L_):
            P = plan(l)
            direct_tasks(P)
            direct_first = fork is not None and bool(P.tasks)
            if direct_first:
                fork.run(3, lambda: launch_direct(P))
            stage_a(P, "lar", forked=fork)
            mark("conv_prep")
            launch_factorised(P)
            join_lists()
            if direct_first:
                fork.join()
            else:
                launch_direct(P)
            mark("conv_launch")
            fix_rowmaps(P)
            if dbg is not None:
                for k, ent in P.msgs.items():
                    n_k = nodes[RECV_TYPE[k]][1]
                    o_k = torch.zeros((n_k, P.spec.d_out), device=dev)
                    K.launch_reduce(o_k, P.spec.d_out, n_k, P.spec.d_out, [ent], accumulate=False)
                    dbg[f"conv_layers.{9 * l + k}"] = o_k
            if fork is not None and m.fork_small_means:
                fork.run(0, lambda: means(P, "l"))
                fork.run(1, lambda: means(P, "r"))
                means(P, "a")
                fork.join()
            else:
                means(P, "lar")
            mark("reduce")
            F.keep.append((P.keep, P.per, P.msgs, P.tasks, P.tasks_g, P.gmap))

    def _heads(self, data, S, F, lig, rec, atom, dev, mark):
        m = self.m
        ns, L_, B, ldx = m.ns, m.num_conv_layers, S.B, m._ldx
        Nl, Na = S.Nl, S.Na
        xl, xa, lpos = F.xl, F.xa, F.lpos
        lay_l, lay_a, lbatch, abatch = S.lay_l, S.lay_a, S.lbatch, S.abatch
        tr_sigma, rot_sigma, tor_sigma, sc_sigma = F.sig
        if m.confidence_mode:
            def scalars(x):
                return torch.cat([x[:, :ns], x[:, m._d_final - ns:m._d_final]], dim=1) if L_ >= 3 else x[:, :ns]

            def graph_mean(v, b):
                lay = G.DenseLayout.build(b, B)
                return lay.dense(v, 0.0).sum(1) / lay.counts.clamp(min=1).unsqueeze(1)

            conf_in = lay_l.dense(scalars(xl), 0.0).sum(1) / lay_l.counts.clamp(min=1).unsqueeze(1)
            if m.flexible_sidechains:
                if S.num_flex > 0:
                    fr = data["flexResidues"]
                    bonds = lay_a.starts[fr.batch.long()] + fr.edge_idx.t().long()
                    flex_atoms = torch.unique(bonds)
                    conf_in = torch.cat([conf_in, graph_mean(scalars(xa)[flex_atoms], abatch[flex_atoms])], dim=1)
                else:
                    conf_in = torch.cat([conf_in, torch.zeros_like(conf_in)], dim=1)
            return m.confidence_predictor(conf_in).squeeze(dim=-1)

        dd = m.distance_embed_dim
        lib = L.load()
# ... 87 lines not shown
```

diffdock_pocket_amd/launch.py:

```python
from __future__ import annotations

import ctypes as C
import os
from dataclasses import dataclass
from typing import Dict, List, NamedTuple, Optional, Sequence

import torch
from torch import nn

from . import _lib as L
from . import packing as P
from .graph import EdgeView


def require_hip(t: torch.Tensor):
    if not t.is_cuda:
        raise L.DdpError("the MI355X score model runs on a HIP device only (no CPU/eager fallback); "
                         "move the batch to cuda:<n>")
    L.load()


def stream():
    return C.c_void_p(torch._C._cuda_getCurrentRawStream(torch._C._cuda_getDevice()))

# ... 33 lines not shown
class ConvProfiler:

    def __init__(self):
        self.events, self.kernel, self.specs, self.counts, self.node_bytes, self.tags, self.h2 = [], [], [], [], [], [], []
        self.hbm = {}
        self.hbm_on = False
        self._resolved = None

    def record_conv(self, e0, e1, spec, flops_spec, tasks_counts, node_bytes, tag=None, h2=False, rows=False):
        self.events.append((e0, e1))
        self.tags.append(tag)
        self.h2.append(bool(h2))
        self.kernel.append((("ddp_conv_rows16_kernel" if spec.factorized else "ddp_conv_rows16_direct_kernel") if int(rows) == 2 else "ddp_conv_rows_kernel") if rows else
                           "ddp_conv32_kernel" if spec.factorized else "ddp_conv_messages_kernel")
        self.specs.append((spec, flops_spec or spec))
        self.counts.append(tasks_counts)
        self.node_bytes.append(node_bytes)
        self._resolved = None

    def _resolve(self):
        if self._resolved is None:
            torch.cuda.synchronize()
            cache = {}

            def val(cap, cnt):
                if cnt is None:
                    return cap
                key = (cnt.data_ptr(), id(cnt))
                if key not in cache:
                    cache[key] = min(cap, max(0, int(cnt.item())))
                return cache[key]

            ne = [sum(val(c, t) for c, t in tc) for tc in self.counts]
            self.edges = ne
            self.flops = [fs.flops_per_edge() * n for (s, fs), n in zip(self.specs, ne)]
            self.executed = [(s.mfma_flops_per_edge_executed() + 2 * s.hid * sum(s.g_cols)) * n for (s, fs), n in zip(self.specs, ne)]
            self.useful = [s.useful_flops_per_edge() * n for (s, fs), n in zip(self.specs, ne)]
            self.fc = [(s.fc_flops_per_edge() + (2 * s.hid * sum(s.g_cols) if k.startswith("ddp_conv_rows") else 0)) * n
                       for (s, fs), n, k in zip(self.specs, ne, self.kernel)]
            self.boundary = [n * (4.0 * fs.f_in + 32.0) + nb for (s, fs), n, nb in zip(self.specs, ne, self.node_bytes)]
            self._resolved = True

    def hbm_summary(self, name):
        rec = self.hbm.get(name, [])
        torch.cuda.synchronize()
        return len(rec), float(sum((r[2]() if callable(r[2]) else r[2]) for r in rec)), float(sum(r[0].elapsed_time(r[1]) for r in rec))

    def summary(self, kernel=None):
        self._resolve()
        sel = [i for i, k in enumerate(self.kernel) if kernel is None or k == kernel]
        ms = sum(self.events[i][0].elapsed_time(self.events[i][1]) for i in sel)
        return len(sel), float(sum(self.flops[i] for i in sel)), float(ms)

    def split_flops(self, kernel=None, tag=False):
        self._resolve()
        fc16 = sum(f for f, k, h in zip(self.fc, self.kernel, self.h2) if h and (kernel is None or k == kernel))
        useful = sum(u for u, k in zip(self.useful, self.kernel) if kernel is None or k == kernel)
        return float(fc16), float(useful - fc16)

    def by_tag(self, kernel):
        self._resolve()
        out = {}
        for i, k in enumerate(self.kernel):
            if k != kernel:
                continue
            n, u, ms, ne, f16 = out.get(self.tags[i], (0, 0.0, 0.0, 0, 0.0))
            out[self.tags[i]] = (n + 1, u + self.useful[i], ms + self.events[i][0].elapsed_time(self.events[i][1]), ne + self.edges[i],
                                 f16 + (self.fc[i] if self.h2[i] else 0.0))
        return out

    def executed_flops(self, kernel=None):
        self._resolve()
        return float(sum(e for e, k in zip(self.executed, self.kernel) if kernel is None or k == kernel))

    def useful_flops(self, kernel=None):
        self._resolve()
        return float(sum(e for e, k in zip(self.useful, self.kernel) if kernel is None or k == kernel))

    def boundary_bytes(self):
        self._resolve()
        return float(sum(self.boundary))


_PROFILER: Optional[ConvProfiler] = None


def set_conv_profiler(p: Optional[ConvProfiler]):
    global _PROFILER
    _PROFILER = p


def profiler(hbm=False) -> Optional[ConvProfiler]:
    p = _PROFILER
    if p is not None and hbm and not p.hbm_on:
        return None
    return p


class SectionTimer:

    def __init__(self):
        self.marks = []

    def mark(self, name):
        import time
        ev = torch.cuda.Event(enable_timing=True)
        ev.record()
        self.marks.append((name, ev, time.perf_counter()))

    def summary(self):
        torch.cuda.synchronize()
        out = {}
        for (n0, e0, t0), (n1, e1, t1) in zip(self.marks[:-1], self.marks[1:]):
            if n1 == "start":
                continue
            g, h = out.get(n1, (0.0, 0.0))
            out[n1] = (g + e0.elapsed_time(e1), h + (t1 - t0) * 1e3)
        return out


CONV_H2 = True
_RANGE_FLAG = None


def set_range_flag(t):
    global _RANGE_FLAG
    _RANGE_FLAG = t


CONV_ROWS = os.environ.get("DDP_CONV_ROWS", "1") != "0"


def occupancy_shaping(rows_min_lds: int = 0, stage_a_pad: int = 0):
    L.check(L.load().ddp_set_occupancy_shaping(int(rows_min_lds), int(stage_a_pad)), "ddp_set_occupancy_shaping")


class ConvPath(NamedTuple):
    rows: bool
    h2: bool
    rows_form: int = 0
    gh_fmt: int = 0
    rows_bias_k: int = 0
    rows_seg: tuple = (0, 0)
    rows_nts: int = 0


def conv_path(pk, rows_ok: bool = True) -> ConvPath:
    h2 = CONV_H2 and pk.w1h is not None and pk.w2h is not None
    if not (CONV_H2 and CONV_ROWS and rows_ok and pk.wsh is not None):
        return ConvPath(False, h2)
    return ConvPath(True, h2, pk.rows_form, pk.gh_fmt, pk.rows_bias_k, pk.rows_seg, pk.rows_nts)


def make_task(pk, path: ConvPath, x_src, ldx_src, view: EdgeView, sh, segs, msg, g=None) -> L.ConvTask:
    t = L.ConvTask()
    t.x_src, t.ldx_src, t.n_edges = x_src.data_ptr(), ldx_src, view.n_edges
    t.src, t.eid, t.sh = view.src.data_ptr(), view.eid.data_ptr(), sh.data_ptr()
    for k in range(L.DDP_MAX_SEGS):
        if k < len(segs):
            ten, idx, ld, n = segs[k]
            t.seg_ptr[k], t.seg_idx[k], t.seg_ld[k], t.seg_n[k] = ten.data_ptr(), idx.data_ptr(), ld, n
        else:
            t.seg_ptr[k], t.seg_idx[k], t.seg_ld[k], t.seg_n[k] = 0, 0, 0, 0
    t.w1p, t.b1p, t.w2p, t.b2p = pk.w1p.data_ptr(), pk.b1p.data_ptr(), pk.w2p.data_ptr(), pk.b2p.data_ptr()
    t.w1h, t.w2h = (pk.w1h.data_ptr(), pk.w2h.data_ptr()) if path.h2 else (0, 0)
    t.h2_range_flag = _p(_RANGE_FLAG) if path.h2 else 0
    t.msg = msg.data_ptr()
    t.wsh, t.bsp = (pk.wsh.data_ptr(), pk.bsp.data_ptr()) if path.rows else (0, 0)
    for k in range(2):
        gk = g[k].data_ptr() if (g is not None and g[k] is not None) else 0
        t.g[k], t.gh[k] = (0, gk) if path.rows else (gk, 0)
    t.gh_fmt, t.rows_form, t.rows_bias_k, t.rows_nts = path.gh_fmt, path.rows_form, path.rows_bias_k, path.rows_nts
    t.rows_seg0, t.rows_seg1 = path.rows_seg
    t._path = path
    t.pos = _p(view.pos)
    t.n_edges_dev = _p(view.cnt)
    t._count = (view.n_edges, view.cnt)
    return t


def launch_convs(spec: P.ConvSpec, tasks: List[L.ConvTask], flops_spec: Optional[P.ConvSpec] = None, node_bytes: float = 0.0, tag=None):
    lib = L.load()
    if not tasks:
        return
    path = tasks[0]._path
    if any((t._path.rows, t._path.rows_form) != (path.rows, path.rows_form) for t in tasks):
        raise L.DdpError("launch_convs: the tasks of one launch run through different conv kernels")
    arr = (L.ConvTask * len(tasks))(*tasks)
    shape = spec.ctypes_shape()
    prof = _PROFILER
    if prof is not None:
        e0, e1 = torch.cuda.Event(enable_timing=True), torch.cuda.Event(enable_timing=True)
        e0.record()
    if path.rows:
        L.check(lib.ddp_conv_rows(C.byref(shape), arr, len(tasks), stream()), "ddp_conv_rows")
    else:
        L.check(lib.ddp_conv_messages(C.byref(shape), arr, len(tasks), stream()), "ddp_conv_messages")
    if prof is not None:
        e1.record()
        h2 = P.h2_steps(spec) > 0 and all(t._path.h2 for t in tasks)
        prof.record_conv(e0, e1, spec, flops_spec, [t._count for t in tasks], node_bytes, tag, h2,
                         rows=(2 if path.rows_form == 1 else 1) if path.rows else 0)


def launch_reduce(x, ldx, n_nodes, d_out, sources, accumulate=True, n_rep=1, rep_stride=0):
    lib = L.load()
    arr = (L.ReduceSrc * max(len(sources), 1))()
    for i, src_ in enumerate(sources):
        msg, view, pk = src_[:3]
        arr[i].msg, arr[i].rowptr = msg.data_ptr(), view.rowptr.data_ptr()
        arr[i].bn_scale, arr[i].bn_shift, arr[i].n_edges = pk.bn_scale.data_ptr(), pk.bn_shift.data_ptr(), view.n_edges
        arr[i].rowmap = src_[3].data_ptr() if (len(src_) > 3 and src_[3] is not None) else 0
        arr[i].n_edges_dev = _p(view.cnt)
    prof = profiler(hbm=True)
    if prof is not None:
        e0, e1 = torch.cuda.Event(enable_timing=True), torch.cuda.Event(enable_timing=True)
        e0.record()
    L.check(lib.ddp_segment_reduce(ptr(x), ldx, n_nodes, d_out, arr, len(sources), 1 if accumulate else 0, n_rep, rep_stride,
                                   stream()), "ddp_segment_reduce")
    if prof is not None:
        e1.record()
        views = [s_[1] for s_ in sources]

        def nbytes(views=views, d_out=d_out, n_nodes=n_nodes, n_rep=n_rep):
            ne = sum(v.n_edges if v.cnt is None else min(v.n_edges, int(v.cnt.item())) for v in views)
            return 4.0 * d_out * (ne + 2 * n_nodes * max(n_rep, 1))
        wide = (d_out % 4 == 0 and ldx % 4 == 0 and x.data_ptr() % 16 == 0 and not os.environ.get("DDP_REDUCE_NARROW")
                and all(s_[0].data_ptr() % 16 == 0 and s_[2].bn_scale.data_ptr() % 16 == 0 and s_[2].bn_shift.data_ptr() % 16 == 0 for s_ in sources))
        prof.hbm.setdefault("ddp_segment_reduce4_kernel" if wide else "ddp_segment_reduce_kernel", []).append((e0, e1, nbytes))


class EdgeMLPPack:

    def __init__(self, seq: nn.Sequential, rbf_slice: slice, device):
        W1, b1, W2, b2 = seq[0].weight.detach(), seq[0].bias.detach(), seq[3].weight.detach(), seq[3].bias.detach()
        ns = W1.shape[0]
        k = rbf_slice.stop - rbf_slice.start
        w1d = torch.zeros(k, 64, device=device)
        w1d[:, :ns] = W1[:, rbf_slice].t()
        w2 = torch.zeros(64, 64, device=device)
        w2[:ns, :ns] = W2.t()
        b2p = torch.zeros(64, device=device)
        b2p[:ns] = b2
        self.w1d, self.w2, self.b2, self.ns, self.k = w1d.contiguous(), w2.contiguous(), b2p, ns, k
        self.W1, self.b1 = W1, b1


def edge_featurize(pack: EdgeMLPPack, dist, pos_a, ia, pos_b, ib, pre, pre_idx, pre2=None, n_edges=None, cnt=None):
    lib = L.load()
    E = int(ia.shape[0]) if n_edges is None else int(n_edges)
    dev = pos_a.device
    out = torch.empty((E, pack.ns), device=dev, dtype=torch.float32)
    sh = torch.empty((E, 4), device=dev, dtype=torch.float32)
    if E == 0:
        return out, sh
    if pre.stride(1) != 1:
        pre = pre.contiguous()
    n2 = 0 if pre2 is None else int(pre2.shape[0])
    L.check(lib.ddp_edge_featurize(ptr(pos_a), ptr(ia), ptr(pos_b), ptr(ib), E, ptr(cnt), ptr(dist.offset), pack.k,
                                   C.c_float(dist.coeff), ptr(pre), ptr(pre_idx), pre.stride(0),
                                   ptr(pre2) if n2 else None, n2, pre2.stride(0) if n2 else 0, ptr(pack.w1d),
                                   ptr(pack.w2), ptr(pack.b2), pack.ns, ptr(out), ptr(sh), stream()),
            "ddp_edge_featurize")
    return out, sh


def edge_featurize_jobs(calls):
    if any(a[0].k % 8 or not 8 <= a[0].k <= 64 for a, _ in calls) or len(calls) > L.DDP_MAX_FEATURIZE_JOBS:
        return [edge_featurize(*a, **kw) for a, kw in calls]
    jobs, outs, keep = [], [], []
    for (pack, dist, pos_a, ia, pos_b, ib, pre, pre_idx), kw in calls:
        pre2, n_edges, cnt = kw.get("pre2"), kw.get("n_edges"), kw.get("cnt")
        E = int(ia.shape[0]) if n_edges is None else int(n_edges)
        out = torch.empty((E, pack.ns), device=pos_a.device, dtype=torch.float32)
        sh = torch.empty((E, 4), device=pos_a.device, dtype=torch.float32)
        outs.append((out, sh))
        if E == 0:
            continue
        if pre.stride(1) != 1:
            pre = pre.contiguous()
        n2 = 0 if pre2 is None else int(pre2.shape[0])
        j = L.FeaturizeJob()
        j.pos_a, j.ia, j.pos_b, j.ib, j.n_edges, j.n_edges_dev = _p(pos_a), _p(ia), _p(pos_b), _p(ib), E, _p(cnt)
        j.offset, j.k_rbf, j.coeff = _p(dist.offset), pack.k, float(dist.coeff)
        j.pre, j.pre_idx, j.ld_pre = _p(pre), _p(pre_idx), pre.stride(0)
        j.pre2, j.n_pre2, j.ld_pre2 = (_p(pre2) if n2 else 0), n2, (pre2.stride(0) if n2 else 0)
        j.w1d, j.w2, j.b2, j.ns, j.out, j.sh = _p(pack.w1d), _p(pack.w2), _p(pack.b2), pack.ns, _p(out), _p(sh)
        jobs.append(j)
        keep.append((pre, pre2, ia, ib, pre_idx))
    if jobs:
        arr = (L.FeaturizeJob * len(jobs))(*jobs)
        L.check(L.load().ddp_edge_featurize_jobs(arr, len(jobs), stream()), "ddp_edge_featurize_jobs")
    return outs


@dataclass
class StageAStack:
    W: torch.Tensor
    meta: list
    offs: object
    path: ConvPath
    gh: Optional[torch.Tensor]
    ld: int
    Wh: Optional[torch.Tensor] = None
    W3: Optional[torch.Tensor] = None

    def prepare(self, h2: bool, x3: bool) -> "StageAStack":
        if (h2 or self.path.rows) and self.Wh is None:
            self.Wh = P.split_h2(self.W, unified_scale=P.GH_SW) if self.path.rows else P.split_h2(self.W)
        if x3 and not self.path.rows and self.W3 is None:
            self.W3 = P.split_bf16x3(self.W)
        return self


def stage_a_stack(packs, hid: int, path: ConvPath) -> StageAStack:
    Ws, meta, ghs, lds = [], [], [], set()
    for key, pk in packs:
        for slot in (0, 1):
            if pk.wg[slot] is None:
                continue
            meta.append((key, slot, pk.g_in_off[slot]))
            Ws.append(pk.wgh[slot] if path.rows else pk.wg[slot])
            if path.rows:
                ghs.append(pk.gh_groups[slot])
                lds.add(pk.gh_ld[slot])
    assert len(lds) <= 1, "the convs of one stage-A launch write G rows of one length"
    W = torch.stack(Ws).contiguous()
    gh = torch.stack([P.gh_dest_table(ws, (hid + 7) // 8, W.shape[2], fmt=path.gh_fmt) for ws in ghs]).contiguous().to(W.device) if path.rows else None
    return StageAStack(W, meta, (C.c_int32 * len(meta))(*[mm[2] for mm in meta]), path, gh, lds.pop() if lds else W.shape[2])


def stage_a(x, n_rows, st: StageAStack, out, rows=None, rows_cnt=None, out_rows=None, h2=False, x3=False):
    lib = L.load()
    nb, n_in, ncols = st.W.shape
    if nb > L.DDP_MAX_GEMM_BATCH:
        raise L.DdpError("more (conv, slot) pairs per source array than DDP_MAX_GEMM_BATCH")
    if n_rows == 0:
        return
    args = (x.data_ptr(), x.stride(0), n_rows, ptr(rows), ptr(rows_cnt), out_rows if out_rows is not None else n_rows, st.offs, nb,
            st.W.data_ptr())
    if st.path.rows:
        fn, name = (lib.ddp_stage_a_gh3, "ddp_stage_a_gh3") if st.path.gh_fmt == 1 else (lib.ddp_stage_a_gh, "ddp_stage_a_gh")
        L.check(fn(*args, ptr(st.Wh), n_in, ncols, out.data_ptr(), st.ld, ptr(_RANGE_FLAG), st.gh.data_ptr(), stream()), name)
    elif h2:
        L.check(lib.ddp_stage_a_h2(*args, ptr(st.Wh), n_in, ncols, out.data_ptr(), ncols, ptr(_RANGE_FLAG), stream()), "ddp_stage_a_h2")
    else:
        L.check(lib.ddp_stage_a(*args, ptr(st.W3 if x3 else None), n_in, ncols, out.data_ptr(), ncols, stream()), "ddp_stage_a")

# ... 528 lines not shown
```

diffdock_pocket_amd/packing.py:

```python
from __future__ import annotations

import math
import os
from dataclasses import dataclass, field
from typing import List, Sequence, Tuple

import torch

from . import _lib as L


@dataclass
class BlockSpec:
    U: int
    n: int
    C: int
    out_off: int
    w_off: int
    scale: float
    segs: List[Tuple[int, int, int]]
    tile0: int = 0
    ntiles: int = 0
    nsub: int = 1
    ups: int = 1
# ... 329 lines not shown
        return 0
    return {180: 12, 96: 6, 72: 5, 48: 3}.get(spec.hid, 0)


def _pack_tiles_h2(Wcols: torch.Tensor, ns16: int, unified_scale: float = 0.0) -> torch.Tensor:
    ncols, K = Wcols.shape
    kp = 16 * ns16
    assert ncols % 32 == 0 and kp >= K
    W = torch.zeros(ncols, kp, dtype=torch.float32)
    W[:, :K] = Wcols
    if unified_scale > 0.0:
        W = W * unified_scale
    hi = W.to(torch.float16)
    lo = ((W - hi.float()) * (1.0 if unified_scale > 0.0 else H2_SCALE)).to(torch.float16)
    if not bool(torch.isfinite(hi).all()):
        raise NotImplementedError("fc weight outside the fp16 range (|w| > 65504, ddp_conv_rows' planes: |w| > 255): the fp16 hi/lo form cannot "
                                  "represent it")
    Pl = torch.stack([hi, lo], 0).reshape(2, ncols // 32, 32, ns16, 2, 8)
    return Pl.permute(1, 3, 0, 4, 2, 5).contiguous().reshape(-1)


def rows16_pos(ncols: int) -> torch.Tensor:
    c = torch.arange(ncols)
    j = c % 32
    return (c - j) + 16 * ((j & 7) >> 2) + 4 * (j >> 3) + (j & 3)


def _pack_tiles_16(Wcols: torch.Tensor, ns16: int, unified_scale: float) -> torch.Tensor:
    ncols, K = Wcols.shape
    kp = 16 * ns16
    assert ncols % 32 == 0 and kp >= K and ns16 % 2 == 0
    W = torch.zeros(ncols, kp, dtype=torch.float32)
    W[:, :K] = Wcols
    W = W * unified_scale
    hi = W.to(torch.float16)
    lo = (W - hi.float()).to(torch.float16)
    if not bool(torch.isfinite(hi).all()):
        raise NotImplementedError("fc weight outside the fp16 range of ddp_conv_rows' planes (|w| > 255): the fp16 hi/lo form cannot represent it")
    Pl = torch.stack([hi, lo], 0).reshape(2, ncols // 32, 2, 16, ns16 // 2, 4, 8)
    return Pl.permute(1, 4, 2, 0, 5, 3, 6).contiguous().reshape(-1)


def pack_fc1_h2(spec: ConvSpec, weight: torch.Tensor):
    hid, f_in = weight.shape
    Wc = torch.zeros(spec.nct1 * 32, f_in)
    Wc[:hid] = weight.detach().float().cpu()
    return _pack_tiles_h2(Wc, h2_steps(spec))


def pack_fc2_h2(spec: ConvSpec, weight: torch.Tensor):
    weight = weight.detach().float().cpu()
    cols = []
    for b in spec.blocks:
        rows = b.column_rows()
        valid = rows >= 0
        Wc = torch.zeros(rows.numel(), spec.hid)
        Wc[valid] = weight[rows[valid]] * b.scale
        cols.append(Wc)
    return _pack_tiles_h2(torch.cat(cols, 0), h2_steps(spec))


def pack_fc1(spec: ConvSpec, weight: torch.Tensor, bias: torch.Tensor):
    hid, f_in = weight.shape
    assert (hid, f_in) == (spec.hid, spec.f_in)
    ncols = spec.nct1 * 32
    Wc = torch.zeros(ncols, f_in)
    Wc[:hid] = weight.detach().float().cpu()
    b = torch.zeros(ncols)
    b[:hid] = bias.detach().float().cpu()
    return _pack_tiles(Wc, spec.kp1), b


def pack_fc2(spec: ConvSpec, weight: torch.Tensor, bias: torch.Tensor):
    wn, hid = weight.shape
    assert hid == spec.hid and wn == spec.weight_numel, (weight.shape, spec.weight_numel, spec.hid)
    weight = weight.detach().float().cpu()
    bias = bias.detach().float().cpu()
    cols, bcols = [], []
    for b in spec.blocks:
        rows = b.column_rows()
        valid = rows >= 0
        Wc = torch.zeros(rows.numel(), hid)
        Wc[valid] = weight[rows[valid]] * b.scale
        bc = torch.zeros(rows.numel())
        bc[valid] = bias[rows[valid]] * b.scale
        cols.append(Wc)
        bcols.append(bc)
    return _pack_tiles(torch.cat(cols, 0), spec.hp), torch.cat(bcols, 0)


def bn_affine(out_mul_blocks: Sequence[Tuple[int, int, bool]], running_mean, running_var, weight, bias, eps=1e-5):
    scale_c = (weight.detach().double() / torch.sqrt(running_var.detach().double() + eps))
    scales, shifts, iw, ib = [], [], 0, 0
    for mul, dim, is_scalar in out_mul_blocks:
        s = scale_c[iw:iw + mul]
        scales.append(s.repeat_interleave(dim))
        if is_scalar:
            sh = bias.detach().double()[ib:ib + mul] - running_mean.detach().double()[ib:ib + mul] * s
            ib += mul
        else:
            sh = torch.zeros(mul, dtype=torch.float64)
        shifts.append(sh.repeat_interleave(dim))
        iw += mul
    return torch.cat(scales).float(), torch.cat(shifts).float()

def spec_form1_chunks(spec: "ConvSpec") -> bool:
    return not spec.factorized


def rows_bias_in_k(spec: "ConvSpec") -> bool:
    return (not spec.factorized) and spec.hid % 16 != 0


def rows_supported(spec: "ConvSpec") -> bool:
    ns16 = h2_steps(spec)
    if ns16 not in (12, 6) or (not spec.factorized and not rows_bias_in_k(spec)):
        return False
    for b in spec.blocks:
        if b.C not in (1, 3) or b.n < 1 or b.n > 64 or (b.C == 3 and b.n > 32):
            return False
        if b.nsub < 1 or b.nsub > 2 or b.ups < 1 or (b.nsub > 1) != (b.n > 32) or (b.nsub == 1 and b.ups != 32 // b.n):
            return False
    frows = max([b.U * b.C for b in spec.blocks if b.U > 0] + [0])
    if spec_form1_chunks(spec):
        frows = min(frows, 72)
    priv = max((frows * 36 * 4 + 127) // 128 * 128 + 1408 + 2048, ns16 * 1024)
    nts = spec.nct1 if rows_bias_in_k(spec) else spec.nct1 + sum(len(t) for _, _, t in rows_segments(spec))
    return 2 * (2 * ns16 * 1024 + (nts * 128 + 127) // 128 * 128 + 4 * ((priv + 127) // 128 * 128)) <= 160 * 1024


def rows_kperm(ns16: int) -> torch.Tensor:
    ks = torch.arange(ns16).reshape(-1, 1, 1)
    hh = torch.arange(2).reshape(1, -1, 1)
    i = torch.arange(8).reshape(1, 1, -1)
    j = 8 * (ks % 2) + i
    return (32 * (ks // 2) + (j % 4) + 8 * (j // 4) + 4 * hh).reshape(-1)


def rows_segments(spec: "ConvSpec"):
    segs = []
    for bi, b in enumerate(spec.blocks):
        nparts = (b.n + 31) // 32
        for part in range(nparts):
            if b.U == 0:
                tiles = []
            elif b.nsub > 1:
                tiles = [b.tile0 + u * b.nsub + part for u in range(b.U)]
            else:
                tiles = [b.tile0 + t for t in range((b.U + b.ups - 1) // b.ups)]
            segs.append((bi, part, tiles))
    return segs


def rows_split_segments(spec: "ConvSpec", nsplit: int):
    import itertools
    counts = [len(t) for _, _, t in rows_segments(spec)]
    n = len(counts)
    nsplit = max(1, min(nsplit, n))
    best = None
    for cuts in itertools.combinations(range(1, n), nsplit - 1):
        edges = (0,) + cuts + (n,)
        sums = [sum(counts[a:b]) for a, b in zip(edges[:-1], edges[1:])]
        if best is None or max(sums) < best[0]:
            best = (max(sums), edges, sums)
    _, edges, sums = best
    return [(a, b, c) for a, b, c in zip(edges[:-1], edges[1:], sums)]


def rows_stream(spec: "ConvSpec", w1: torch.Tensor, b1: torch.Tensor, w2: torch.Tensor, b2: torch.Tensor, form: int = 0, bias_in_k: bool = False,
                seg_range=None):
    ns16 = h2_steps(spec)
    assert ns16 > 0
    hid, f_in = w1.shape
    assert not bias_in_k or (form == 1 and hid < 16 * ns16 and hid < spec.nct1 * 32)
    W1c = torch.zeros(spec.nct1 * 32, f_in)
    W1c[:hid] = w1.detach().float().cpu()
    b1c = torch.zeros(spec.nct1 * 32)
    b1c[:hid] = b1.detach().float().cpu() * (ROWS_SW * ROWS_SX)
    if bias_in_k:
        b1c[hid] = 1.0 * (ROWS_SW * ROWS_SX)
    if form == 1:
        pos = rows16_pos(spec.nct1 * 32)
        W1p, b1p = torch.zeros_like(W1c), torch.zeros_like(b1c)
        W1p[pos] = W1c
        b1p[pos] = b1c
        W1c, b1c = W1p, b1p
        t1 = _pack_tiles_16(W1c, ns16, ROWS_SW).reshape(spec.nct1, -1)
    else:
        t1 = _pack_tiles_h2(W1c, ns16, ROWS_SW).reshape(spec.nct1, -1)
    w2 = w2.detach().float().cpu()
    b2 = b2.detach().float().cpu()
    cols, bcols = [], []
    for b in spec.blocks:
        rows = b.column_rows()
        valid = rows >= 0
        Wc = torch.zeros(rows.numel(), spec.hid)
        Wc[valid] = w2[rows[valid]] * b.scale
        bc = torch.zeros(rows.numel())
        bc[valid] = b2[rows[valid]] * b.scale
        cols.append(Wc)
        bcols.append(bc)
    segs = rows_segments(spec)
    if seg_range is not None:
        segs = segs[seg_range[0]:seg_range[1]]
    order = [t for _, _, tiles in segs for t in tiles]
    if order:
        Wall = torch.cat(cols, 0)
        Wp = torch.zeros(Wall.shape[0], 16 * ns16)
        Wp[:, :spec.hid] = Wall
        if bias_in_k:
            Wp[:, spec.hid] = torch.cat(bcols, 0)
        if form == 1:
            t2 = _pack_tiles_16(Wp, ns16, ROWS_SW).reshape(Wall.shape[0] // 32, -1)[order]
        else:
            Wp = Wp[:, rows_kperm(ns16)]
            t2 = _pack_tiles_h2(Wp, ns16, ROWS_SW).reshape(Wall.shape[0] // 32, -1)[order]
        bs2 = torch.cat(bcols, 0).reshape(-1, 32)[order] * (0.0 if bias_in_k else ROWS_SH * ROWS_SW)
        return torch.cat([t1, t2], 0).reshape(-1).contiguous(), torch.cat([b1c.reshape(-1, 32), bs2], 0).contiguous()
    return t1.reshape(-1).contiguous(), b1c.reshape(-1, 32).contiguous()


def gh_parts(spec: "ConvSpec", slot: int):
    parts, cum = [], 0
    for bi, b in enumerate(spec.blocks):
        if b.g_slot != slot:
            continue
        for part in range((b.n + 31) // 32):
            w = min(32, b.n - 32 * part)
            wp = (w + 3) // 4 * 4
            parts.append((bi, part, b.g_col0 + 32 * part, w, wp, cum))
            cum += wp
    return parts


def gh_ld(hid: int, gcp: int) -> int:
    return (((hid + 7) // 8 * 8 + 1) * gcp + 31) // 32 * 32


GH3_FP32_COLS = (0, 1, 4, 5, 2, 6)


def gh3_ld(hid: int, gcp: int) -> int:
    n8 = (hid + 7) // 8
    return (n8 * gcp + (gcp + 5) // 6 + 15) // 16 * 96


def factor_weights_gh(spec: "ConvSpec", weight: torch.Tensor, bias: torch.Tensor, fmt: int = 0, form: int = 0):
    ns16 = h2_steps(spec)
    assert ns16 > 0
    weight = weight.detach().float().cpu()
    bias = bias.detach().float().cpu()
    n8 = (spec.hid + 7) // 8
    kp = torch.arange(8 * n8) if form == 1 else rows_kperm(ns16)[:8 * n8]
    Wg, offs, widths = [None, None], [0, 0], [None, None]
    for slot in (0, 1):
        blks = [b for b in spec.blocks if b.g_slot == slot]
        if not blks:
            continue
        gc = spec.g_cols[slot]
        n_in = blks[0].g_count
        assert all(b.g_count == n_in and b.g_in_off == blks[0].g_in_off for b in blks)
        W = torch.zeros(n_in, 16 * ns16, gc)
        Bm = torch.zeros(n_in, gc)
        for b in blks:
            rows = b.w_off + (b.g_u0 + torch.arange(n_in)).reshape(-1, 1) * b.n + torch.arange(b.n).reshape(1, -1)
            W[:, :spec.hid, b.g_col0:b.g_col0 + b.n] = (weight[rows] * b.scale).permute(0, 2, 1)
            Bm[:, b.g_col0:b.g_col0 + b.n] = bias[rows] * b.scale
        parts = gh_parts(spec, slot)
        gcp = sum(p[4] for p in parts)
        ld = gh_ld(spec.hid, gcp) if fmt != 1 else gh3_ld(spec.hid, gcp) // 6 * 8
        Wfull = torch.zeros(n_in, ld)
        Wk = W[:, kp].reshape(n_in, n8, 8, gc)
        for _, _, c0, w, wp, cum in parts:
            tile = torch.zeros(n_in, n8, wp, 8)
            tile[:, :, :w] = Wk[:, :, :, c0:c0 + w].permute(0, 1, 3, 2) * ROWS_SG
            Wfull[:, 8 * n8 * cum:8 * n8 * (cum + wp)] = tile.reshape(n_in, -1)
            if fmt != 1:
                Wfull[:, 8 * n8 * gcp + cum:8 * n8 * gcp + cum + w] = Bm[:, c0:c0 + w] * (ROWS_SH * ROWS_SG)
            else:
                cpad = cum + torch.arange(w)
                Wfull[:, 8 * n8 * gcp + 8 * (cpad // 6) + torch.tensor(GH3_FP32_COLS)[cpad % 6]] = Bm[:, c0:c0 + w] * (ROWS_SH * ROWS_SG)
        Wg[slot], offs[slot], widths[slot] = Wfull.contiguous(), blks[0].g_in_off, [p[4] for p in parts]
    return Wg, offs, widths


def gh_dest_table(widths: Sequence[int], n8: int, ncols: int, fmt: int = 0) -> torch.Tensor:
    ng = ncols // 8
    tab = torch.empty((ng, 2), dtype=torch.int32)
    g = torch.arange(ng, dtype=torch.int64)
    if fmt == 1:
        gcp = sum(widths)
        assert 8 * (n8 * gcp + (gcp + 5) // 6) <= ncols and ncols % 128 == 0
        tab[:, 0] = (6 * g).int()
        tab[:, 1] = (6 * g + 4).int()
        tab[:n8 * gcp, 0] += 1
        return tab
    tab[:, 0] = (8 * g).int()
    tab[:, 1] = (8 * g + 4).int()
    cum = 0
    for w in widths:
        gs = n8 * cum
        gl = torch.arange(n8 * w, dtype=torch.int64)
        unit = 2 * (gs + gl)
        tab[gs:gs + n8 * w, 0] = (4 * unit + 1).int()
        tab[gs:gs + n8 * w, 1] = (4 * (unit + 1)).int()
        cum += w
    assert 8 * n8 * cum + cum <= ncols
    return tab
```

diffdock_pocket_amd/score_model.py:

```python
from __future__ import annotations

import math
import os
from typing import Dict, List, Optional

import numpy as np
import torch
from torch import nn

from . import _lib as L
from . import graph as G
from . import launch as K
from . import packing as P
from .synthetic import LIG_FEATURE_DIMS, REC_ATOM_FEATURE_DIMS, REC_RESIDUE_FEATURE_DIMS

ASSETS = os.path.join(os.path.dirname(os.path.abspath(__file__)), "assets")


class GaussianSmearing(nn.Module):

    def __init__(self, start=0.0, stop=5.0, num_gaussians=50):
        super().__init__()
        offset = torch.linspace(start, stop, num_gaussians)
        self.coeff = -0.5 / (offset[1] - offset[0]).item() ** 2
        self.register_buffer("offset", offset)


class AtomEncoder(nn.Module):

    def __init__(self, emb_dim, feature_dims, sigma_embed_dim, lm_embedding_type=None):
        super().__init__()
        self.num_categorical_features = len(feature_dims)
        if lm_embedding_type is not None and lm_embedding_type != "esm":
            raise ValueError("LM Embedding type was not correctly determined. LM embedding type: ", lm_embedding_type)
        lm_dim = 1280 if lm_embedding_type == "esm" else 0
        self.additional_features_dim = sigma_embed_dim + lm_dim
        self.atom_embedding_list = nn.ModuleList()
        for dim in feature_dims:
            emb = nn.Embedding(dim, emb_dim)
            nn.init.xavier_uniform_(emb.weight.data)
            self.atom_embedding_list.append(emb)
        if self.additional_features_dim > 0:
            self.additional_features_embedder = nn.Linear(self.additional_features_dim + emb_dim, emb_dim)

    def forward(self, x_cat, extra):
        emb = 0
        for i in range(self.num_categorical_features):
            emb = emb + self.atom_embedding_list[i](x_cat[:, i].long())
        if self.additional_features_dim > 0:
            emb = self.additional_features_embedder(torch.cat([emb, extra], dim=1))
        return emb

    def forward_split(self, x_cat, static_extra, sigma_emb, cached):
        lin = self.additional_features_embedder
        n_static = lin.in_features - sigma_emb.shape[1]

        def static():
            emb = 0
            for i in range(self.num_categorical_features):
                emb = emb + self.atom_embedding_list[i](x_cat[:, i].long())
            feats = emb if static_extra is None else torch.cat([emb, static_extra.float()], dim=1)
            return torch.nn.functional.linear(feats, lin.weight[:, :n_static], lin.bias)

        return cached(static) + sigma_emb @ lin.weight[:, n_static:].t()


class OldAtomEncoder(nn.Module):

    def __init__(self, emb_dim, feature_dims, sigma_embed_dim, lm_embedding_type=None):
        super().__init__()
        self.num_categorical_features = len(feature_dims)
        self.num_scalar_features = sigma_embed_dim
        self.lm_embedding_type = lm_embedding_type
        self.atom_embedding_list = nn.ModuleList()
        for dim in feature_dims:
            emb = nn.Embedding(dim, emb_dim)
            nn.init.xavier_uniform_(emb.weight.data)
            self.atom_embedding_list.append(emb)
        if self.num_scalar_features > 0:
            self.linear = nn.Linear(self.num_scalar_features, emb_dim)
        if lm_embedding_type is not None:
            if lm_embedding_type != "esm":
                raise ValueError("LM Embedding type was not correctly determined. LM embedding type: ", lm_embedding_type)
            self.lm_embedding_dim = 1280
            self.lm_embedding_layer = nn.Linear(self.lm_embedding_dim + emb_dim, emb_dim)

    def forward(self, x_cat, extra):
        emb = 0
        for i in range(self.num_categorical_features):
            emb = emb + self.atom_embedding_list[i](x_cat[:, i].long())
        if self.num_scalar_features > 0:
            emb = emb + self.linear(extra[:, :self.num_scalar_features])
        if self.lm_embedding_type is not None:
            emb = self.lm_embedding_layer(torch.cat([emb, extra[:, -self.lm_embedding_dim:]], dim=1))
        return emb


class IrrepsBatchNorm(nn.Module):

    def __init__(self, blocks):
        super().__init__()
        self.blocks = list(blocks)
        n_scalar = sum(m for m, _, s in blocks if s)
        n_feat = sum(m for m, _, _ in blocks)
        self.register_buffer("running_mean", torch.zeros(n_scalar))
        self.register_buffer("running_var", torch.ones(n_feat))
        self.weight = nn.Parameter(torch.ones(n_feat))
        self.bias = nn.Parameter(torch.zeros(n_scalar))


def _mlp(n_in, n_hidden, n_out, dropout):
    return nn.Sequential(nn.Linear(n_in, n_hidden), nn.ReLU(), nn.Dropout(dropout), nn.Linear(n_hidden, n_out))


class _PackedConv:
    __slots__ = ("w1p", "b1p", "w2p", "b2p", "bn_scale", "bn_shift", "wg", "bg", "g_in_off", "w1h", "w2h",
                 "wsh", "bsp", "wgh", "gh_groups", "gh_ld", "gh_fmt", "rows_form", "rows_bias_k", "rows_seg", "rows_nts")

    def __init__(self, **fields):
        self.wg = self.bg = self.g_in_off = self.w1h = self.w2h = None
        self.wsh = self.bsp = self.wgh = self.gh_groups = self.gh_ld = None
        self.gh_fmt = self.rows_form = self.rows_bias_k = self.rows_nts = 0
        self.rows_seg = (0, 0)
        for k, v in fields.items():
            setattr(self, k, v)


G_PLANES3_DEFAULT = "1"
DIRECT_ROWS_DEFAULT = "1"
ROWS_MFMA16_DEFAULT = "1"


def rows_defaults():
    env = os.environ.get
    return (env("DDP_ROWS_MFMA16", ROWS_MFMA16_DEFAULT) == "1", env("DDP_G_PLANES3", G_PLANES3_DEFAULT) == "1",
            env("DDP_DIRECT_ROWS", DIRECT_ROWS_DEFAULT) == "1")


class TensorProductConvLayer(nn.Module):

    def __init__(self, spec: P.ConvSpec, out_blocks, batch_norm=True, dropout=0.0, spec_g: Optional[P.ConvSpec] = None):
        super().__init__()
        self.spec = spec
        self.spec_g = spec_g
        self.out_blocks = list(out_blocks)
        self.fc = _mlp(spec.f_in, spec.hid, spec.weight_numel, dropout)
        self.batch_norm = IrrepsBatchNorm(out_blocks) if batch_norm else None
        self._packed: Optional[_PackedConv] = None
        self._packed_g: Optional[_PackedConv] = None
        self._packed_d = None
        rows16, planes3, self.direct_rows = rows_defaults()
        self.rows_form, self.gh_fmt = int(rows16), int(planes3)

    def packed_g(self, device) -> _PackedConv:
        if self._packed_g is None or self._packed_g.w1p.device != device:
            base = self.packed(device)
            w2p, b2p = P.pack_fc2(self.spec_g, self.fc[3].weight, self.fc[3].bias)
            if w2p.numel() == 0:
                w2p, b2p = torch.zeros(64), torch.zeros(32)
            pk = _PackedConv(w1p=base.w1p, b1p=base.b1p, bn_scale=base.bn_scale, bn_shift=base.bn_shift, w1h=base.w1h,
                             w2p=w2p.to(device), b2p=b2p.to(device), gh_fmt=self.gh_fmt, rows_form=self.rows_form)
            if P.h2_steps(self.spec_g) > 0:
                w2h = P.pack_fc2_h2(self.spec_g, self.fc[3].weight)
                pk.w2h = (w2h if w2h.numel() else torch.zeros(64, dtype=torch.float16)).to(device)
            wg, bg, offs = P.factor_weights(self.spec_g, self.fc[3].weight, self.fc[3].bias)
            pk.wg = [w.to(device) if w is not None else None for w in wg]
            pk.bg = [b.to(device) if b is not None else None for b in bg]
            pk.g_in_off = offs
            if P.rows_supported(self.spec_g):
                try:
                    wsh, bsp = P.rows_stream(self.spec_g, self.fc[0].weight, self.fc[0].bias, self.fc[3].weight, self.fc[3].bias, form=pk.rows_form)
                    wgh, _, widths = P.factor_weights_gh(self.spec_g, self.fc[3].weight, self.fc[3].bias, fmt=pk.gh_fmt, form=pk.rows_form)
                    for w in wgh:
                        if w is not None:
                            P.split_h2(w.unsqueeze(0), unified_scale=P.GH_SW)
                except NotImplementedError:
                    wsh = None
                if wsh is not None:
                    pk.wsh, pk.bsp = wsh.to(device), bsp.to(device)
                    pk.wgh = [w.to(device) if w is not None else None for w in wgh]
                    pk.gh_groups = widths
                    pk.gh_ld = [None if w is None else (P.gh3_ld(self.spec_g.hid, sum(ws)) if pk.gh_fmt == 1 else w.shape[1])
                                for w, ws in zip(wgh, widths)]
            self._packed_g = pk
        return self._packed_g

    def node_tensors(self, pk: _PackedConv, x_src: torch.Tensor, path: K.ConvPath):
        N = x_src.shape[0]
        st = K.stage_a_stack([(0, pk)], self.spec_g.hid, path).prepare(h2=False, x3=False)
        out = torch.empty((len(st.meta), N, st.ld), device=x_src.device, dtype=torch.float32)
        K.stage_a(x_src, N, st, out)
        g = [None, None]
        for i, (_, slot, _) in enumerate(st.meta):
            g[slot] = out[i]
        return g

    def packed(self, device) -> _PackedConv:
        if self._packed is None or self._packed.w1p.device != device:
            w1p, b1p = P.pack_fc1(self.spec, self.fc[0].weight, self.fc[0].bias)
            w2p, b2p = P.pack_fc2(self.spec, self.fc[3].weight, self.fc[3].bias)
            if self.batch_norm is not None:
                bn = self.batch_norm
                sc, sh = P.bn_affine(self.out_blocks, bn.running_mean.cpu(), bn.running_var.cpu(), bn.weight.cpu(), bn.bias.cpu())
            else:
                sc, sh = torch.ones(self.spec.d_out), torch.zeros(self.spec.d_out)
            pk = _PackedConv(w1p=w1p.to(device), b1p=b1p.to(device), w2p=w2p.to(device), b2p=b2p.to(device),
                             bn_scale=sc.to(device), bn_shift=sh.to(device))
            if P.h2_steps(self.spec) > 0:
                pk.w1h = P.pack_fc1_h2(self.spec, self.fc[0].weight).to(device)
                pk.w2h = P.pack_fc2_h2(self.spec, self.fc[3].weight).to(device)
            self._packed = pk
            self._packed_d = None
        return self._packed

    def packed_rows_direct(self, device, nsplit: int = 1):
        base = self.packed(device)
        if not (self.direct_rows and self.rows_form == 1 and not self.spec.factorized and P.rows_supported(self.spec)):
            return None
        if self._packed_d is None or self._packed_d[0] is not base:
            self._packed_d = (base, {})
        cache = self._packed_d[1]
        ranges = P.rows_split_segments(self.spec, nsplit) if nsplit > 1 else [None]
        key = len(ranges)
        if key not in cache:
            pks = []
            for rg in ranges:
                pk = _PackedConv(**{name: getattr(base, name) for name in ("w1p", "b1p", "w2p", "b2p", "bn_scale", "bn_shift", "w1h", "w2h")},
                                 rows_form=1, rows_bias_k=1)
                if rg is not None:
                    pk.rows_seg, pk.rows_nts = (rg[0], rg[1]), self.spec.nct1 + rg[2]
                try:
                    wsh, bsp = P.rows_stream(self.spec, self.fc[0].weight, self.fc[0].bias, self.fc[3].weight, self.fc[3].bias, form=1, bias_in_k=True,
                                             seg_range=None if rg is None else (rg[0], rg[1]))
                    pk.wsh, pk.bsp = wsh.to(device), bsp.to(device)
                    pks.append(pk)
                except NotImplementedError:
                    pks = None
                    break
            cache[key] = pks
        pks = cache[key]
        if pks is None:
            return None
        return pks if nsplit > 1 else pks[0]

    def messages(self, node_attr, edge_index, edge_attr, edge_sh, out_nodes=None, factorized=False):
        _require_hip(node_attr)
        dev = node_attr.device
        n_out = int(out_nodes) if out_nodes is not None else node_attr.shape[0]
        csr = G.build_csr(edge_index[0].long(), edge_index[1].long(), n_out)
        x = node_attr.float().contiguous()
        ea = edge_attr.float().contiguous()
        sh = edge_sh.float().contiguous()
        if sh.shape[1] != 4:
            raise NotImplementedError("edge_sh must be [E,4] (lmax=1) or pre-contracted torsion harmonics [0,t]")
        msg = (torch.empty if self.spec.covers_output() else torch.zeros)((csr.n_edges, self.spec.d_out), device=dev, dtype=torch.float32)
        if factorized:
            if self.spec_g is None:
                raise NotImplementedError("this conv has no factorised variant")
            pk, view = self.packed_g(dev), G.source_order(csr, x.shape[0])
            path = K.conv_path(pk, rows_ok=ea.shape[1] % 12 == 0)
            g = self.node_tensors(pk, x, path)
        else:
            pk, view, g = self.packed_rows_direct(dev) if ea.shape[1] % 12 == 0 else None, csr, None
            if pk is None or not K.conv_path(pk).rows:
                pk = self.packed(dev)
            path = K.conv_path(pk)
        if path.rows:
            w3 = ea.shape[1] // 3
            segs = [(ea[:, i * w3:], view.eid, ea.shape[1], w3) for i in range(3)]
        else:
            segs = [(ea, view.eid, ea.shape[1], ea.shape[1])]
        task = _make_task(pk, path, x, x.shape[1], view, sh, segs, msg, g=g)
        _launch_convs(self.spec_g if factorized else self.spec, [task], flops_spec=self.spec if factorized else None)
        return msg, csr, path

    def forward(self, node_attr, edge_index, edge_attr, edge_sh, out_nodes=None, reduce="mean", edge_weight=1.0,
                factorized=False):
        if reduce != "mean" or not (isinstance(edge_weight, (int, float)) and edge_weight == 1.0):
            raise NotImplementedError("HIP conv implements reduce='mean', edge_weight=1")
        if edge_index.numel() == 0:
            return torch.tensor(0, dtype=node_attr.dtype, device=node_attr.device)
        msg, csr, _ = self.messages(node_attr, edge_index, edge_attr, edge_sh, out_nodes=out_nodes, factorized=factorized)
        dev = node_attr.device
        n_out = int(out_nodes) if out_nodes is not None else node_attr.shape[0]
        out = torch.zeros((n_out, self.spec.d_out), device=dev, dtype=torch.float32)
        _launch_reduce(out, self.spec.d_out, n_out, self.spec.d_out, [(msg, csr, self.packed(dev))], accumulate=False)
        return out


_require_hip, _stream, _ptr = K.require_hip, K.stream, K.ptr
ConvProfiler, SectionTimer, set_conv_profiler = K.ConvProfiler, K.SectionTimer, K.set_conv_profiler
_EdgeMLPPack, _edge_featurize = K.EdgeMLPPack, K.edge_featurize
_make_task, _launch_convs, _launch_reduce = K.make_task, K.launch_convs, K.launch_reduce


class _EncoderPack:

    def __init__(self, enc, dev):
        tabs = [e.weight.detach().float() for e in enc.atom_embedding_list]
        self.table = torch.cat(tabs, 0).contiguous().to(dev)
        self.feat_off = [0]
        for t in tabs[:-1]:
            self.feat_off.append(self.feat_off[-1] + t.shape[0])
        self.n_cat, self.emb_dim = len(tabs), tabs[0].shape[1]
        self.old = isinstance(enc, OldAtomEncoder)
        if self.old:
            self.has_lm = enc.lm_embedding_type is not None
            self.n_scalar = enc.num_scalar_features
            if self.n_scalar > 0:
                self.w1, self.b1 = enc.linear.weight.detach().float().t().contiguous().to(dev), enc.linear.bias.detach().float().to(dev)
            if self.has_lm:
                lin = enc.lm_embedding_layer
                self.w2, self.b2 = lin.weight.detach().float().t().contiguous().to(dev), lin.bias.detach().float().to(dev)
        else:
            self.has_extra = enc.additional_features_dim > 0
            if self.has_extra:
                lin = enc.additional_features_embedder
                self.w, self.b = lin.weight.detach().float().t().contiguous().to(dev), lin.bias.detach().float().to(dev)


def _node_job(n_rows, out, ncols, w, bias, zero_to=0, cat=None, pack=None, emb_mode=0, dense=(), sigma=None, sig_out=None, add=None):
    j = L.NodeJob()
    j.n_rows, j.out, j.ld_out, j.ncols, j.zero_to = n_rows, out.data_ptr(), out.stride(0), ncols, zero_to
    j.w, j.bias = w.data_ptr(), (bias.data_ptr() if bias is not None else 0)
    if cat is not None and emb_mode:
        j.cat, j.ld_cat, j.n_cat, j.table, j.emb_dim, j.emb_mode = cat.data_ptr(), cat.stride(0), pack.n_cat, pack.table.data_ptr(), pack.emb_dim, emb_mode
        for f, o in enumerate(pack.feat_off):
            j.feat_off[f] = o
    for d, (ten, c0, n) in enumerate(dense):
        j.dense[d], j.ld_dense[d], j.n_dense[d] = ten.data_ptr() + 4 * c0, ten.stride(0), n
    if sigma is not None and sigma[0] == "t":
        _, t, scale, freq, sd = sigma
        j.t, j.t_stride, j.scale, j.freq, j.sd = t.data_ptr(), (t.stride(0) if t.numel() > 1 else 0), scale, freq.data_ptr(), sd
    elif sigma is not None:
        j.sig_emb, j.ld_sig, j.sd = sigma[1].data_ptr(), sigma[1].stride(0), sigma[1].shape[1]
    if sig_out is not None:
        j.sig_out, j.ld_sig_out = sig_out.data_ptr(), sig_out.stride(0)
    if add is not None:
# ... 517 lines not shown
```

include/ddp_hip.h:

```cpp
#ifndef DDP_HIP_H
#define DDP_HIP_H

#include <stdint.h>

#ifdef __cplusplus
extern "C" {
#endif

#define DDP_ABI_VERSION 17
#define DDP_EINVAL (-1)
#define DDP_ELIMIT (-2)

#define DDP_MAX_TASKS 9
#define DDP_MAX_BLOCKS 4
#define DDP_MAX_SEGS 3
#define DDP_MAX_NS 64
#define DDP_EDGE_TILE 64

enum ddp_feat_kind {
  DDP_F_SCALAR_S0 = 0,
  DDP_F_DOT = 1,
  DDP_F_SCALAR_S1 = 2,
  DDP_F_VEC_S0 = 3,
  DDP_F_CROSS = 4
};

typedef struct {
  int32_t kind;
  int32_t in_off;
  int32_t count;
} ddp_seg_t;

typedef struct {
  int32_t U;
  int32_t n;
  int32_t C;
  int32_t out_off;
  int32_t tile0;
  int32_t ntiles;
  int32_t nsub;
  int32_t ups;
  int32_t nseg;
  ddp_seg_t seg[DDP_MAX_SEGS];
  int32_t g_slot;
  int32_t g_col0;
} ddp_block_t;

#define DDP_CONV32_WAVES 4
#define DDP_MAX_ROLE_SEGS 2
typedef struct {
  int32_t block, tile0, tstride, count, round;
} ddp_role_seg_t;

typedef struct {
  int32_t f_in;
  int32_t hid;
  int32_t kp1;
  int32_t hp;
  int32_t hs;
  int32_t nct1;
  int32_t d_out;
  int32_t nblocks;
  int32_t fbuf_floats;
  int32_t g_cols[2];
  ddp_block_t blk[DDP_MAX_BLOCKS];
  int32_t nrounds;
  int32_t nrole[DDP_CONV32_WAVES];
  ddp_role_seg_t role[DDP_CONV32_WAVES][DDP_MAX_ROLE_SEGS];
} ddp_conv_shape_t;

typedef struct {
  const float* x_src;
  int32_t ldx_src;
  int32_t n_edges;
  const int32_t* src;
  const int32_t* eid;
  const float* sh;
  const float* seg_ptr[DDP_MAX_SEGS];
  const int32_t* seg_idx[DDP_MAX_SEGS];
  int32_t seg_ld[DDP_MAX_SEGS];
  int32_t seg_n[DDP_MAX_SEGS];
  const float* w1p;
  const float* b1p;
  const float* w2p;
  const float* b2p;
  float* msg;
  const float* g[2];
  const int32_t* pos;
  const int32_t* n_edges_dev;
  const void* w1h;
  const void* w2h;
  int32_t* h2_range_flag;
  const void* wsh;
  const float* bsp;
  const void* gh[2];
  int32_t gh_fmt;
  int32_t rows_form;
  int32_t rows_bias_k;
  int32_t rows_seg0, rows_seg1, rows_nts;
} ddp_conv_task_t;
#define DDP_ROWS_SX 16
#define DDP_ROWS_SW 256
#define DDP_ROWS_SH 16
#define DDP_ROWS_SG 32
#define DDP_ROWS_KPERM(ks, hh, i) (32 * ((ks) >> 1) + ((8 * ((ks) & 1) + (i)) & 3) + 8 * ((8 * ((ks) & 1) + (i)) >> 2) + 4 * (hh))
#define DDP_ROWS16_POS(j) (16 * (((j) & 7) >> 2) + 4 * ((j) >> 3) + ((j) & 3))
#define DDP_GH3_LD(hid, gcp) ((((((hid) + 7) / 8) * (gcp) + ((gcp) + 5) / 6 + 15) / 16) * 96)
#define DDP_GH_LD(hid, gcp) ((((((hid) + 7) / 8) * 8 + 1) * (gcp) + 31) / 32 * 32)
int ddp_conv_messages(const ddp_conv_shape_t* shape, const ddp_conv_task_t* tasks, int ntasks, void* stream);

int ddp_conv_rows(const ddp_conv_shape_t* shape, const ddp_conv_task_t* tasks, int ntasks, void* stream);

typedef struct {
  const float* msg;
  const int32_t* rowptr;
  const float* bn_scale;
  const float* bn_shift;
  int32_t n_edges;
  const int32_t* rowmap;
  const int32_t* n_edges_dev;
} ddp_reduce_src_t;
int ddp_segment_reduce(float* x, int ldx, int n_nodes, int d_out, const ddp_reduce_src_t* srcs, int nsrc,
                       int accumulate, int n_rep, int rep_stride, void* stream);

int ddp_edge_featurize(const float* pos_a, const int32_t* ia, const float* pos_b, const int32_t* ib, int n_edges,
                       const int32_t* n_edges_dev, const float* offset, int k_rbf, float coeff, const float* pre,
                       const int32_t* pre_idx, int ld_pre, const float* pre2, int n_pre2, int ld_pre2, const float* w1d,
                       const float* w2, const float* b2, int ns, float* out, float* sh, void* stream);

#define DDP_MAX_FEATURIZE_JOBS 8
typedef struct {
  const float* pos_a;
  const int32_t* ia;
  const float* pos_b;
  const int32_t* ib;
  int32_t n_edges;
  const int32_t* n_edges_dev;
  const float* offset;
  int32_t k_rbf;
  float coeff;
  const float* pre;
  const int32_t* pre_idx;
  int32_t ld_pre;
  const float* pre2;
  int32_t n_pre2, ld_pre2;
  const float* w1d;
  const float* w2;
  const float* b2;
  int32_t ns;
  float* out;
  float* sh;
} ddp_featurize_job_t;
int ddp_edge_featurize_jobs(const ddp_featurize_job_t* jobs, int njobs, void* stream);

int ddp_torsion_sh(const float* sh_edge, const float* bond_vec, const int32_t* bond_of_edge, int n_edges,
                   const int32_t* n_edges_dev, float* out, const float* x, int ldx, int ns, const int32_t* b0,
                   const int32_t* b1, int n_bonds, float* bond_attr, void* stream);

typedef struct {
  const float* t[4];
  int32_t t_stride[4];
  float sig_min[4], sig_max[4];
  float* sigma[4];
  int32_t n_graphs;
  float* cut;
  float cut_mul, cut_add;
  float* graph_emb;
  int32_t sd;
  float emb_scale;
  const float* freq;
  const float* lig_pos;
  const int32_t* graph_ptr;
  float* center;
  struct {
    const float* pos;
    const int32_t* b0;
    const int32_t* b1;
    int32_t n;
    float* mid;
    float* vec;
  } bonds[2];
  struct {
    const int32_t* src;
    int32_t* dst;
    int32_t n;
  } copy[2];
} ddp_prologue_args_t;
int ddp_step_prologue(const ddp_prologue_args_t* args, void* stream);

typedef struct {
  const float* gp;
  int32_t ld_gp, n_graphs, ns, sd;
  const float* graph_emb;
  const float* w1[2];
  const float* b1[2];
  const float* w2[2];
  const float* b2[2];
  const float* sigma[2];
  const float* so3_table;
  int32_t so3_n;
  float so3_lo, so3_span;
  float* out[2];
} ddp_trrot_args_t;
int ddp_trrot_head(const ddp_trrot_args_t* args, void* stream);

typedef struct {
  const float* h;
  int32_t ld_h, n_bonds, ns;
  const float* w1;
  const float* w2;
  const float* sigma;
  const int32_t* graph_of_bond;
  const float* torus_table;
  int32_t torus_n;
  float torus_lo, torus_span;
  float* out;
} ddp_tor_args_t;
int ddp_tor_head(const ddp_tor_args_t* args, void* stream);

#define DDP_MAX_GEMM_BATCH 16
#define DDP_G_LD(hid, gcols) ((((((hid) + 3) / 4) * 4 + 1) * (gcols) + 31) / 32 * 32)
int ddp_stage_a(const float* x, int ldx, int nrows, const int32_t* rows, const int32_t* nrows_dev, int out_rows, const int32_t* offs,
                int nbatch, const float* w, const void* w_bf16x3, int k, int ncols, float* out, int ldo, void* stream);

int ddp_stage_a_h2(const float* x, int ldx, int nrows, const int32_t* rows, const int32_t* nrows_dev, int out_rows, const int32_t* offs,
                   int nbatch, const float* w, const void* w_h2, int k, int ncols, float* out, int ldo, int32_t* range_flag, void* stream);
int ddp_stage_a_gh(const float* x, int ldx, int nrows, const int32_t* rows, const int32_t* nrows_dev, int out_rows, const int32_t* offs,
                   int nbatch, const float* w, const void* w_h2, int k, int ncols, float* out, int ldo, int32_t* range_flag,
                   const int32_t* dest, void* stream);

int ddp_stage_a_gh3(const float* x, int ldx, int nrows, const int32_t* rows, const int32_t* nrows_dev, int out_rows, const int32_t* offs,
                    int nbatch, const float* w, const void* w_h2, int k, int ncols, float* out, int ldo, int32_t* range_flag,
                    const int32_t* dest, void* stream);

#define DDP_GH_SX 2

int ddp_set_occupancy_shaping(int rows_min_lds_bytes, int stage_a_lds_pad_bytes);

extern int ddp_sa_drainwave;

extern int ddp_conv_deal;
int ddp_conv_deal_tile(int id, int total, int c);

int ddp_pose_update(const float* pos_in, int n_samples, int n_atoms, const float* tr, const float* rot, const float* tor,
                    int n_tor, const int32_t* bonds, const uint8_t* mask_rotate, float* pos_out, void* stream);

int ddp_sidechain_update(const float* pos_in, int n_samples, int n_atoms, const float* angles, int n_bonds,
                         const int32_t* edge_idx, const int32_t* subcomponents, const int32_t* mapping, float* pos_out,
                         void* stream);

typedef struct {
  const float* score[4];
  const float* z[4];
  float* out[4];
  int32_t n[4];
} ddp_sde_args_t;
int ddp_sde_update(const float* coef, const ddp_sde_args_t* args, void* stream);

#define DDP_RADIUS_DROP_SELF 1
#define DDP_RADIUS_NEAREST 2
int ddp_radius_count(const float* x, const int32_t* x_ptr, const float* y, const int32_t* y_batch, int ny, float r,
                     int max_neighbors, int flags, int32_t* counts, void* stream);
int ddp_radius_fill(const float* x, const int32_t* x_ptr, const float* y, const int32_t* y_batch, int ny, float r,
                    int max_neighbors, int flags, const int32_t* offsets, int32_t* out_query, int32_t* out_x, void* stream);
int ddp_knn(const float* x, const int32_t* x_ptr, const int32_t* batch, int n, int k, int32_t* out_neighbors, void* stream);
// ... 433 lines not shown
```

Before: 178.3.

## Split row-stationary conv tasks across output segment ranges when the grid underfills the GPU

```diff
diff --git a/diffdock_pocket_amd/_lib.py b/diffdock_pocket_amd/_lib.py
--- a/diffdock_pocket_amd/_lib.py
+++ b/diffdock_pocket_amd/_lib.py
@@ -19,7 +19,7 @@
 DDP_SCORE_GUIDANCE_FLEX_MAX_ATOMS, DDP_SCORE_GUIDANCE_FLEX_MAX_TORSIONS = DDP_MINIMIZE_MAX_ATOMS, DDP_GUIDANCE_MAX_TORSIONS
 DDP_SCORE_GUIDANCE_FLEX_MAX_MOVING, DDP_SCORE_GUIDANCE_FLEX_MAX_BONDS = DDP_MINIMIZE_FLEX_MAX_MOVING, DDP_MINIMIZE_FLEX_MAX_BONDS
 DDP_PAIRWISE_MAX_SAMPLES, DDP_CLUSTER_MAX_SAMPLES = 32768, 1024
-EXPORTS = ["ddp_conv_messages", "ddp_conv_rows", "ddp_stage_a_gh", "ddp_stage_a_gh3", "ddp_segment_reduce", "ddp_edge_featurize", "ddp_edge_featurize_jobs", "ddp_torsion_sh", "ddp_stage_a", "ddp_stage_a_h2",
+EXPORTS = ["ddp_conv_messages", "ddp_conv_rows", "ddp_conv_rows_split", "ddp_conv_rows_split_plan", "ddp_stage_a_gh", "ddp_stage_a_gh3", "ddp_segment_reduce", "ddp_edge_featurize", "ddp_edge_featurize_jobs", "ddp_torsion_sh", "ddp_stage_a", "ddp_stage_a_h2",
            "ddp_pose_update", "ddp_sidechain_update", "ddp_sde_update", "ddp_radius_count", "ddp_radius_fill", "ddp_knn", "ddp_group_by_key", "ddp_node_linear", "ddp_scan_jobs", "ddp_mark_jobs", "ddp_rowcopy_jobs", "ddp_select_jobs",
            "ddp_gather_rows", "ddp_clean_pair_maps", "ddp_flex_mark", "ddp_fallback_rowmap", "ddp_step_prologue", "ddp_trrot_head", "ddp_tor_head", "ddp_radius_search_jobs", "ddp_group_by_key_jobs", "ddp_set_occupancy_shaping", "ddp_pose_rmsd", "ddp_pose_contacts", "ddp_pose_pairwise_rmsd", "ddp_pose_cluster", "ddp_traj_record", "ddp_svgd_tau", "ddp_svgd_pairs", "ddp_svgd_rows", "ddp_refine_energy", "ddp_refine_direction", "ddp_refine_accept", "ddp_clash_guidance", "ddp_score_guidance", "ddp_score_guidance_flex", "ddp_pose_score", "ddp_pose_profile", "ddp_pose_minimize", "ddp_pose_minimize_flex", "ddp_pose_search", "ddp_pose_search_select", "ddp_pose_search_flex", "ddp_pocket_occupancy", "ddp_pocket_buriedness", "ddp_pocket_label", "ddp_conv_deal_tile", "ddp_abi_version", "ddp_last_error", "ddp_source_hash"]
 
@@ -56,6 +56,24 @@
                 ("b2p", C.c_void_p), ("msg", C.c_void_p), ("g", C.c_void_p * 2),
                 ("pos", C.c_void_p), ("n_edges_dev", C.c_void_p), ("w1h", C.c_void_p), ("w2h", C.c_void_p), ("h2_range_flag", C.c_void_p),
                 ("wsh", C.c_void_p), ("bsp", C.c_void_p), ("gh", C.c_void_p * 2), ("gh_fmt", C.c_int32), ("rows_form", C.c_int32), ("rows_bias_k", C.c_int32), ("rows_seg0", C.c_int32), ("rows_seg1", C.c_int32), ("rows_nts", C.c_int32)]
+
+
+DDP_ROWS_MAX_RANGES, DDP_ROWS_MAX_SETS = 6, 3
+
+
+class RowsRange(C.Structure):
+    _fields_ = [("wsh", C.c_void_p), ("bsp", C.c_void_p), ("seg0", C.c_int32), ("seg1", C.c_int32), ("nts", C.c_int32), ("reserved", C.c_int32)]
+
+
+class RowsSplit(C.Structure):
+    _fields_ = [("nsets", C.c_int32), ("k", C.c_int32 * DDP_ROWS_MAX_SETS), ("ranges", C.POINTER(RowsRange) * DDP_ROWS_MAX_SETS)]
+
+
+def rows_split_switch(value=None):
+    var = C.c_int.in_dll(load(), "ddp_rows_split")
+    if value is not None:
+        var.value = int(value)
+    return var.value
 
 
 class ReduceSrc(C.Structure):
@@ -272,6 +290,10 @@
     lib.ddp_conv_messages.restype = C.c_int
     lib.ddp_conv_rows.argtypes = lib.ddp_conv_messages.argtypes
     lib.ddp_conv_rows.restype = C.c_int
+    lib.ddp_conv_rows_split.argtypes = [C.POINTER(ConvShape), C.POINTER(ConvTask), C.c_int, C.POINTER(RowsSplit), C.c_void_p]
+    lib.ddp_conv_rows_split.restype = C.c_int
+    lib.ddp_conv_rows_split_plan.argtypes = [C.POINTER(ConvShape), C.POINTER(ConvTask), C.c_int, C.POINTER(RowsSplit), C.POINTER(C.c_int32 * 4)]
+    lib.ddp_conv_rows_split_plan.restype = C.c_int
     lib.ddp_segment_reduce.argtypes = [C.c_void_p, C.c_int, C.c_int, C.c_int, C.POINTER(ReduceSrc), C.c_int, C.c_int,
                                        C.c_int, C.c_int, C.c_void_p]
     lib.ddp_segment_reduce.restype = C.c_int
diff --git a/diffdock_pocket_amd/csrc/ddp_conv_rows.hip b/diffdock_pocket_amd/csrc/ddp_conv_rows.hip
--- a/diffdock_pocket_amd/csrc/ddp_conv_rows.hip
+++ b/diffdock_pocket_amd/csrc/ddp_conv_rows.hip
@@ -662,7 +662,124 @@
   }
 }
 
-int ddp_conv_rows_plan(const ddp_conv_shape_t* shape, const ddp_conv_task_t* tasks, int ntasks, RowsPlan* plan) {
+#define DDP_ROWS_SPLIT_DEFAULT 100
+extern "C" int ddp_rows_split;
+int ddp_rows_split = -1;
+static int rows_split_pct(void) {
+  if (ddp_rows_split < 0) {
+    const char* e = getenv("DDP_ROWS_SPLIT");
+    const int v = (e && e[0] >= '0' && e[0] <= '9') ? atoi(e) : DDP_ROWS_SPLIT_DEFAULT;
+    ddp_rows_split = (v == 0) ? 0 : (v < 50 || v > 1000) ? DDP_ROWS_SPLIT_DEFAULT : v;
+  }
+  return ddp_rows_split;
+}
+static int rows_slots(const RowsPlan& P) {
+  static int cus[64];
+  int dev = 0;
+  if (P.form != 1 || hipGetDevice(&dev) != hipSuccess || dev < 0 || dev >= 64) {
+    (void)hipGetLastError();
+    return 0;
+  }
+  if (cus[dev] == 0) {
+    int n = 0;
+    if (hipDeviceGetAttribute(&n, hipDeviceAttributeMultiprocessorCount, dev) != hipSuccess || n <= 0) {
+      (void)hipGetLastError();
+      return 0;
+    }
+    cus[dev] = n;
+  }
+  return cus[dev] * ddp_conv_rows16_resident(P);
+}
+
+static int rows_plan_split(RowsPlan& P, const ddp_rows_split_t* splits, const int* idx) {
+  ConvLaunch& L = P.L;
+  const ddp_conv_shape_t& S = L.shape;
+  int seg_tiles[2 * DDP_MAX_BLOCKS], nseg = 0;
+  for (int b = 0; b < S.nblocks; ++b) {
+    const ddp_block_t& B = S.blk[b];
+    const int cnt = (B.ntiles == 0 || B.U == 0) ? 0 : (B.nsub > 1 ? B.U : (B.U + B.ups - 1) / B.ups);
+    for (int part = 0; part < ((B.n + 31) >> 5); ++part) seg_tiles[nseg++] = cnt;
+  }
+  for (int i = 0; i < L.ntasks; ++i) {
+    const ddp_rows_split_t& X = splits[idx[i]];
+    if (X.nsets < 0 || X.nsets > DDP_ROWS_MAX_SETS) return ddp_fail(DDP_EINVAL, "ddp_conv_rows_split: nsets");
+    for (int s = 0; s < X.nsets; ++s) {
+      const int k = X.k[s];
+      if (k < 2 || k > DDP_ROWS_MAX_RANGES || k > nseg || (s > 0 && k <= X.k[s - 1]) || !X.ranges[s])
+        return ddp_fail(DDP_EINVAL, "ddp_conv_rows_split: k of a partition (2 .. 6, ascending, at most the shape's segments)");
+      int at = 0;
+      for (int r = 0; r < k; ++r) {
+        const ddp_rows_range_t& R = X.ranges[s][r];
+        if (R.seg0 != at || R.seg1 <= R.seg0 || R.seg1 > nseg) return ddp_fail(DDP_EINVAL, "ddp_conv_rows_split: the ranges of a partition cover the segments once, in order");
+        int nt = S.nct1;
+        for (int g = R.seg0; g < R.seg1; ++g) nt += seg_tiles[g];
+        if (R.nts != nt) return ddp_fail(DDP_EINVAL, "ddp_conv_rows_split: range.nts is not nct1 + the stream tiles of its segments");
+        if (!R.wsh || !R.bsp || (reinterpret_cast<size_t>(R.wsh) & 15) || (reinterpret_cast<size_t>(R.bsp) & 15))
+          return ddp_fail(DDP_EINVAL, "ddp_conv_rows_split: range.wsh / bsp missing (or not 16-byte aligned)");
+        at = R.seg1;
+      }
+      if (at != nseg) return ddp_fail(DDP_EINVAL, "ddp_conv_rows_split: the ranges of a partition cover the segments once, in order");
+    }
+  }
+  const int pct = rows_split_pct();
+  if (pct == 0 || P.form != 1 || P.slots <= 0 || P.tiles >= P.slots) return 0;
+  for (int i = 0; i < L.ntasks; ++i)
+    if (L.task[i].rows_seg0 != 0 || L.task[i].rows_seg1 != 0 || L.task[i].rows_nts != 0) return 0;
+  int best = 1, set_of[DDP_MAX_TASKS];
+  for (int k = 2; k <= DDP_ROWS_MAX_RANGES; ++k) {
+    if (k * L.ntasks > DDP_MAX_TASKS || (long long)k * P.tiles * 100 > (long long)P.slots * pct) break;
+    bool all = true;
+    for (int i = 0; i < L.ntasks && all; ++i) {
+      const ddp_rows_split_t& X = splits[idx[i]];
+      bool has = false;
+      for (int s = 0; s < X.nsets; ++s) has = has || X.k[s] == k;
+      all = has;
+    }
+    if (all) best = k;
+  }
+  if (best == 1) return 0;
+  const int k = best;
+  for (int i = 0; i < L.ntasks; ++i) {
+    const ddp_rows_split_t& X = splits[idx[i]];
+    for (int s = 0; s < X.nsets; ++s)
+      if (X.k[s] == k) set_of[i] = s;
+  }
+  int order[DDP_ROWS_MAX_RANGES];
+  for (int r = 0; r < k; ++r) order[r] = r;
+  {
+    const ddp_rows_range_t* R0 = splits[idx[0]].ranges[set_of[0]];
+    for (int a = 1; a < k; ++a)
+      for (int b = a; b > 0 && R0[order[b]].nts > R0[order[b - 1]].nts; --b) {
+        const int t = order[b];
+        order[b] = order[b - 1];
+        order[b - 1] = t;
+      }
+  }
+  ddp_conv_task_t base[DDP_MAX_TASKS];
+  const int nbase = L.ntasks;
+  for (int i = 0; i < nbase; ++i) base[i] = L.task[i];
+  int tiles = 0, n = 0;
+  for (int r = 0; r < k; ++r)
+    for (int i = 0; i < nbase; ++i, ++n) {
+      const ddp_rows_range_t& R = splits[idx[i]].ranges[set_of[i]][order[r]];
+      ddp_conv_task_t& T = L.task[n];
+      T = base[i];
+      T.wsh = R.wsh;
+      T.bsp = R.bsp;
+      T.rows_seg0 = R.seg0;
+      T.rows_seg1 = R.seg1;
+      T.rows_nts = R.nts;
+      L.tile_start[n] = tiles;
+      tiles += (T.n_edges + ROWS_ET - 1) / ROWS_ET;
+    }
+  L.ntasks = n;
+  L.tile_start[n] = tiles;
+  P.tiles = tiles;
+  P.split_k = k;
+  return 0;
+}
+
+int ddp_conv_rows_plan(const ddp_conv_shape_t* shape, const ddp_conv_task_t* tasks, int ntasks, const ddp_rows_split_t* splits, RowsPlan* plan) {
   if (!shape || !tasks) return ddp_fail(DDP_EINVAL, "ddp_conv_rows: null argument");
   if (ntasks < 0 || ntasks > DDP_MAX_TASKS) return ddp_fail(DDP_ELIMIT, "ddp_conv_rows: ntasks > DDP_MAX_TASKS");
   if (shape->nblocks < 1 || shape->nblocks > DDP_MAX_BLOCKS) return ddp_fail(DDP_EINVAL, "ddp_conv_rows: nblocks");
@@ -694,7 +811,7 @@
       if (B.U * B.C > frows) frows = B.U * B.C;
     }
   }
-  int tiles = 0, gfmt = -1, form = -1, bias_k = -1;
+  int tiles = 0, gfmt = -1, form = -1, bias_k = -1, split_idx[DDP_MAX_TASKS];
   for (int i = 0; i < ntasks; ++i) {
     const ddp_conv_task_t& T = tasks[i];
     if (T.n_edges <= 0) continue;
@@ -724,6 +841,7 @@
     if (reinterpret_cast<size_t>(T.sh) & 15) return ddp_fail(DDP_EINVAL, "ddp_conv_rows: sh must be 16-byte aligned");
     L.tile_start[L.ntasks] = tiles;
     L.task[L.ntasks] = T;
+    split_idx[L.ntasks] = i;
     tiles += (T.n_edges + ROWS_ET - 1) / ROWS_ET;
     ++L.ntasks;
   }
@@ -732,6 +850,8 @@
   P.form = form;
   P.gh_fmt = gfmt;
   P.tiles = tiles;
+  P.split_k = 1;
+  P.slots = 0;
   if (tiles == 0) return 0;
   P.nts = nts;
   if (form == 1 && frows > R16_FROWS) frows = R16_FROWS;
@@ -750,12 +870,32 @@
   if (2 * lds_bytes > 160 * 1024) return ddp_fail(DDP_ELIMIT, "ddp_conv_rows: LDS budget of two workgroups per CU exceeded (too many vector features per block)");
   if ((size_t)ddp_shape_rows_min_lds > lds_bytes) lds_bytes = (size_t)ddp_shape_rows_min_lds;
   P.lds_bytes = lds_bytes;
+  if (splits) {
+    P.slots = rows_slots(P);
+    return rows_plan_split(P, splits, split_idx);
+  }
   return 0;
 }
 
+extern "C" int ddp_conv_rows_split_plan(const ddp_conv_shape_t* shape, const ddp_conv_task_t* tasks, int ntasks, const ddp_rows_split_t* splits, int32_t info[4]) {
+  if (!info) return ddp_fail(DDP_EINVAL, "ddp_conv_rows_split_plan: null argument");
+  RowsPlan P;
+  const int rc = ddp_conv_rows_plan(shape, tasks, ntasks, splits, &P);
+  if (rc != 0) return rc;
+  info[0] = P.split_k;
+  info[1] = P.L.ntasks;
+  info[2] = P.tiles;
+  info[3] = (splits || P.tiles == 0) ? P.slots : rows_slots(P);
+  return 0;
+}
+
 extern "C" int ddp_conv_rows(const ddp_conv_shape_t* shape, const ddp_conv_task_t* tasks, int ntasks, void* stream) {
+  return ddp_conv_rows_split(shape, tasks, ntasks, nullptr, stream);
+}
+
+extern "C" int ddp_conv_rows_split(const ddp_conv_shape_t* shape, const ddp_conv_task_t* tasks, int ntasks, const ddp_rows_split_t* splits, void* stream) {
   RowsPlan P;
-  const int rc = ddp_conv_rows_plan(shape, tasks, ntasks, &P);
+  const int rc = ddp_conv_rows_plan(shape, tasks, ntasks, splits, &P);
   if (rc != 0 || P.tiles == 0) return rc;
   if (P.form == 1) return ddp_conv_rows16_launch(P, stream);
   RowsLaunch RL;
diff --git a/diffdock_pocket_amd/csrc/ddp_conv_rows16.hip b/diffdock_pocket_amd/csrc/ddp_conv_rows16.hip
--- a/diffdock_pocket_amd/csrc/ddp_conv_rows16.hip
+++ b/diffdock_pocket_amd/csrc/ddp_conv_rows16.hip
@@ -457,7 +457,7 @@
 
   rows_request_piece<NS>(ring, wsh, 0, ROWS_NP * nts, 0, wave, lane);
   rows_request_piece<NS>(ring, wsh, 1, ROWS_NP * nts, 1, wave, lane);
-  for (int i = tid; i < RL.bias_tiles * 32; i += ROWS_NT) lbias[i] = T.bsp[i];
+  for (int i = tid; i < min(RL.bias_tiles, nts) * 32; i += ROWS_NT) lbias[i] = T.bsp[i];
   h8 xh[NS];
   f32x4* xlo = reinterpret_cast<f32x4*>(priv);
   {
@@ -604,6 +604,33 @@
   r16_body<SZ, 0, true>(RL);
 }
 
+static int r16_lds_have[6] = {0, 0, 0, 0, 0, 0};
+typedef void (*r16_kernel_t)(const R16Launch);
+static r16_kernel_t r16_kernel_of(const RowsPlan& P, int* slot) {
+  const bool direct = P.L.shape.g_cols[0] == 0 && P.L.shape.g_cols[1] == 0;
+  if (direct) return (P.sc == 60) ? (*slot = 4, ddp_conv_rows16_direct_kernel<60>) : (*slot = 5, ddp_conv_rows16_direct_kernel<32>);
+  if (P.sc == 60) return (P.gh_fmt == 1) ? (*slot = 2, ddp_conv_rows16_kernel<60, 1>) : (*slot = 0, ddp_conv_rows16_kernel<60, 0>);
+  return (P.gh_fmt == 1) ? (*slot = 3, ddp_conv_rows16_kernel<32, 1>) : (*slot = 1, ddp_conv_rows16_kernel<32, 0>);
+}
+int ddp_conv_rows16_resident(const RowsPlan& P) {
+  static int for_lds[6] = {0, 0, 0, 0, 0, 0}, resident[6] = {0, 0, 0, 0, 0, 0};
+  int slot = 0;
+  const r16_kernel_t k = r16_kernel_of(P, &slot);
+  if (for_lds[slot] == (int)P.lds_bytes && resident[slot] > 0) return resident[slot];
+  if (ddp_need_lds(reinterpret_cast<const void*>(k), (int)P.lds_bytes, &r16_lds_have[slot]) != hipSuccess) {
+    (void)hipGetLastError();
+    return 0;
+  }
+  int n = 0;
+  if (hipOccupancyMaxActiveBlocksPerMultiprocessor(&n, k, ROWS_NT, P.lds_bytes) != hipSuccess || n <= 0) {
+    (void)hipGetLastError();
+    return 0;
+  }
+  for_lds[slot] = (int)P.lds_bytes;
+  resident[slot] = n;
+  return n;
+}
+
 int ddp_conv_rows16_launch(const RowsPlan& P, void* stream) {
   R16Launch RL;
   RL.L = P.L;
@@ -613,7 +640,7 @@
   RL.priv_bytes = P.priv_bytes;
   RL.aux_off = P.aux_off;
   RL.frows = P.frows;
-  static int lds_have[6] = {0, 0, 0, 0, 0, 0};
+  int (&lds_have)[6] = r16_lds_have;
   hipError_t err;
   const bool direct = P.L.shape.g_cols[0] == 0 && P.L.shape.g_cols[1] == 0;
   if (direct) {
diff --git a/diffdock_pocket_amd/csrc/ddp_conv_rows_common.h b/diffdock_pocket_amd/csrc/ddp_conv_rows_common.h
--- a/diffdock_pocket_amd/csrc/ddp_conv_rows_common.h
+++ b/diffdock_pocket_amd/csrc/ddp_conv_rows_common.h
@@ -167,9 +167,12 @@
   int bias_bytes, priv_bytes, aux_off;
   int frows;
   size_t lds_bytes;
+  int split_k;
+  int slots;
 };
-int ddp_conv_rows_plan(const ddp_conv_shape_t* shape, const ddp_conv_task_t* tasks, int ntasks, RowsPlan* plan);
+int ddp_conv_rows_plan(const ddp_conv_shape_t* shape, const ddp_conv_task_t* tasks, int ntasks, const ddp_rows_split_t* splits, RowsPlan* plan);
 int ddp_conv_rows16_launch(const RowsPlan& P, void* stream);
+int ddp_conv_rows16_resident(const RowsPlan& P);
 
 #define ROWS_LAUNCH(KERNEL_, SLOT_, WHERE_)                                                                          \
   {                                                                                                                  \
diff --git a/diffdock_pocket_amd/engine.py b/diffdock_pocket_amd/engine.py
--- a/diffdock_pocket_amd/engine.py
+++ b/diffdock_pocket_amd/engine.py
@@ -816,6 +816,7 @@
                 conv = m.conv_layers[9 * l + k]
                 pkc = conv.packed(dev)
                 e_base, sh_k = e[ek], sh[ek]
+                rg_ = lambda conv=conv: conv.packed_g_ranges(dev)
                 if k == 3 and c1 is not None:
                     msg = torch.empty((c1.E + c1.e0, spec.d_out), device=dev)
                     P.msgs[k] = (msg, csr, pkc, c1.rowmap)
@@ -823,10 +824,10 @@
                     sd_ = c1.so_d
                     if sd_.n_edges > 0:
                         segs = [(e_base, sd_.eid, ns, ns), (x_recv, sd_.recv, ldx, ns), (xa, sd_.src, ldx, ns)]
-                        tasks_g.append(K.make_task(pkg, path, xa, ldx, sd_, sh_k, segs, msg, g=[P.g_d.get((3, s_)) for s_ in (0, 1)]))
+                        tasks_g.append(K.make_task(pkg, path, xa, ldx, sd_, sh_k, segs, msg, g=[P.g_d.get((3, s_)) for s_ in (0, 1)], ranges=rg_))
                     sv = c1.so_v
                     segs = [(e_base, sv.eid, ns, ns), (P.x_clean, sv.recv, ldx, ns), (P.x_clean, sv.src, ldx, ns)]
-                    tasks_g.append(K.make_task(pkg, path, P.x_clean, ldx, sv, sh_k, segs, msg, g=[P.g_v.get((3, s_)) for s_ in (0, 1)]))
+                    tasks_g.append(K.make_task(pkg, path, P.x_clean, ldx, sv, sh_k, segs, msg, g=[P.g_v.get((3, s_)) for s_ in (0, 1)], ranges=rg_))
                     continue
                 msg = torch.empty((csr.n_edges, spec.d_out), device=dev)
                 P.msgs[k] = (msg, csr, pkc)
@@ -836,7 +837,7 @@
                     nb_g += node_bytes(l, k)
                 segs = [(e_base, so_k.eid, ns, ns), (x_recv, so_k.recv, ldx, ns), (x_src, so_k.src, ldx, ns)]
                 tasks_g.append(K.make_task(conv.packed_g(dev), self._conv_path(conv, dev), x_src, ldx, so_k, sh_k, segs, msg,
-                                           g=[P.gmap.get((k, s_)) for s_ in (0, 1)]))
+                                           g=[P.gmap.get((k, s_)) for s_ in (0, 1)], ranges=rg_))
             P.tasks_g = getattr(P, "tasks_g", []) + tasks_g
             if tasks_g:
                 K.launch_convs(P.spec_g, tasks_g, flops_spec=spec, node_bytes=nb_g, tag=f"layer{l}")
diff --git a/diffdock_pocket_amd/launch.py b/diffdock_pocket_amd/launch.py
--- a/diffdock_pocket_amd/launch.py
+++ b/diffdock_pocket_amd/launch.py
@@ -209,8 +209,9 @@
     return ConvPath(True, h2, pk.rows_form, pk.gh_fmt, pk.rows_bias_k, pk.rows_seg, pk.rows_nts)
 
 
-def make_task(pk, path: ConvPath, x_src, ldx_src, view: EdgeView, sh, segs, msg, g=None) -> L.ConvTask:
+def make_task(pk, path: ConvPath, x_src, ldx_src, view: EdgeView, sh, segs, msg, g=None, ranges=None) -> L.ConvTask:
     t = L.ConvTask()
+    t._ranges = ranges if (path.rows and path.rows_form == 1) else None
     t.x_src, t.ldx_src, t.n_edges = x_src.data_ptr(), ldx_src, view.n_edges
     t.src, t.eid, t.sh = view.src.data_ptr(), view.eid.data_ptr(), sh.data_ptr()
     for k in range(L.DDP_MAX_SEGS):
@@ -236,6 +237,24 @@
     return t
 
 
+def _rows_split_tables(lib, shape, arr, tasks):
+    if not any(getattr(t, "_ranges", None) is not None for t in tasks):
+        return None
+    sw = L.rows_split_switch()
+    if sw == 0 or (sw < 0 and os.environ.get("DDP_ROWS_SPLIT") == "0"):
+        return None
+    info = (C.c_int32 * 4)()
+    L.check(lib.ddp_conv_rows_split_plan(C.byref(shape), arr, len(tasks), None, C.byref(info)), "ddp_conv_rows_split_plan")
+    if not (0 < info[2] < info[3]):
+        return None
+    tabs = (L.RowsSplit * len(tasks))()
+    for i, t in enumerate(tasks):
+        rg = t._ranges() if getattr(t, "_ranges", None) is not None else None
+        if rg is not None:
+            tabs[i] = rg.table
+    return tabs
+
+
 def launch_convs(spec: P.ConvSpec, tasks: List[L.ConvTask], flops_spec: Optional[P.ConvSpec] = None, node_bytes: float = 0.0, tag=None):
     lib = L.load()
     if not tasks:
@@ -250,7 +269,11 @@
         e0, e1 = torch.cuda.Event(enable_timing=True), torch.cuda.Event(enable_timing=True)
         e0.record()
     if path.rows:
-        L.check(lib.ddp_conv_rows(C.byref(shape), arr, len(tasks), stream()), "ddp_conv_rows")
+        tabs = _rows_split_tables(lib, shape, arr, tasks)
+        if tabs is None:
+            L.check(lib.ddp_conv_rows(C.byref(shape), arr, len(tasks), stream()), "ddp_conv_rows")
+        else:
+            L.check(lib.ddp_conv_rows_split(C.byref(shape), arr, len(tasks), tabs, stream()), "ddp_conv_rows_split")
     else:
         L.check(lib.ddp_conv_messages(C.byref(shape), arr, len(tasks), stream()), "ddp_conv_messages")
     if prof is not None:
diff --git a/diffdock_pocket_amd/packing.py b/diffdock_pocket_amd/packing.py
--- a/diffdock_pocket_amd/packing.py
+++ b/diffdock_pocket_amd/packing.py
@@ -505,19 +505,24 @@
     return segs
 
 
-def rows_split_segments(spec: "ConvSpec", nsplit: int):
+ROWS_G_SEGMENT_COST = 3
+
+
+def rows_split_segments(spec: "ConvSpec", nsplit: int, g_cost: int = 0):
     import itertools
-    counts = [len(t) for _, _, t in rows_segments(spec)]
+    segs = rows_segments(spec)
+    counts = [len(t) for _, _, t in segs]
+    costs = [len(t) + (g_cost if spec.blocks[bi].g_slot >= 0 else 0) for bi, _, t in segs]
     n = len(counts)
     nsplit = max(1, min(nsplit, n))
     best = None
     for cuts in itertools.combinations(range(1, n), nsplit - 1):
         edges = (0,) + cuts + (n,)
-        sums = [sum(counts[a:b]) for a, b in zip(edges[:-1], edges[1:])]
+        sums = [sum(costs[a:b]) for a, b in zip(edges[:-1], edges[1:])]
         if best is None or max(sums) < best[0]:
-            best = (max(sums), edges, sums)
-    _, edges, sums = best
-    return [(a, b, c) for a, b, c in zip(edges[:-1], edges[1:], sums)]
+            best = (max(sums), edges)
+    _, edges = best
+    return [(a, b, sum(counts[a:b])) for a, b in zip(edges[:-1], edges[1:])]
 
 
 def rows_stream(spec: "ConvSpec", w1: torch.Tensor, b1: torch.Tensor, w2: torch.Tensor, b2: torch.Tensor, form: int = 0, bias_in_k: bool = False,
diff --git a/diffdock_pocket_amd/score_model.py b/diffdock_pocket_amd/score_model.py
--- a/diffdock_pocket_amd/score_model.py
+++ b/diffdock_pocket_amd/score_model.py
@@ -126,6 +126,36 @@
             setattr(self, k, v)
 
 
+ROWS_SPLIT_KS = (2, 3, 6)
+
+
+class _RowsRanges:
+
+    def __init__(self, base, spec, fc, device, ks=ROWS_SPLIT_KS):
+        self.base, self.sets = base, {}
+        nseg = len(P.rows_segments(spec))
+        self.table = L.RowsSplit()
+        self._arrays = []
+        for k in ks:
+            if k > nseg:
+                continue
+            rgs = P.rows_split_segments(spec, k, g_cost=P.ROWS_G_SEGMENT_COST)
+            if len(rgs) != k:
+                continue
+            arr = (L.RowsRange * k)()
+            rows = []
+            for i, (s0, s1, ntile) in enumerate(rgs):
+                wsh, bsp = P.rows_stream(spec, fc[0].weight, fc[0].bias, fc[3].weight, fc[3].bias, form=base.rows_form, seg_range=(s0, s1))
+                wsh, bsp = wsh.to(device), bsp.to(device)
+                rows.append((wsh, bsp, s0, s1, spec.nct1 + ntile))
+                arr[i].wsh, arr[i].bsp, arr[i].seg0, arr[i].seg1, arr[i].nts = wsh.data_ptr(), bsp.data_ptr(), s0, s1, spec.nct1 + ntile
+            n = self.table.nsets
+            self.table.k[n], self.table.ranges[n] = k, L.C.cast(arr, L.C.POINTER(L.RowsRange))
+            self.table.nsets = n + 1
+            self.sets[k] = rows
+            self._arrays.append(arr)
+
+
 G_PLANES3_DEFAULT = "1"
 DIRECT_ROWS_DEFAULT = "1"
 ROWS_MFMA16_DEFAULT = "1"
@@ -149,6 +179,7 @@
         self._packed: Optional[_PackedConv] = None
         self._packed_g: Optional[_PackedConv] = None
         self._packed_d = None
+        self._packed_gr = None
         rows16, planes3, self.direct_rows = rows_defaults()
         self.rows_form, self.gh_fmt = int(rows16), int(planes3)
 
@@ -184,6 +215,14 @@
                                 for w, ws in zip(wgh, widths)]
             self._packed_g = pk
         return self._packed_g
+
+    def packed_g_ranges(self, device):
+        pk = self.packed_g(device)
+        if pk.wsh is None or pk.rows_form != 1:
+            return None
+        if self._packed_gr is None or self._packed_gr.base is not pk:
+            self._packed_gr = _RowsRanges(pk, self.spec_g, self.fc, device)
+        return self._packed_gr
 
     def node_tensors(self, pk: _PackedConv, x_src: torch.Tensor, path: K.ConvPath):
         N = x_src.shape[0]
diff --git a/include/ddp_hip.h b/include/ddp_hip.h
--- a/include/ddp_hip.h
+++ b/include/ddp_hip.h
@@ -111,6 +111,24 @@
 
 int ddp_conv_rows(const ddp_conv_shape_t* shape, const ddp_conv_task_t* tasks, int ntasks, void* stream);
 
+#define DDP_ROWS_MAX_RANGES 6
+#define DDP_ROWS_MAX_SETS 3
+typedef struct {
+  const void* wsh;
+  const float* bsp;
+  int32_t seg0, seg1;
+  int32_t nts;
+  int32_t reserved;
+} ddp_rows_range_t;
+typedef struct {
+  int32_t nsets;
+  int32_t k[DDP_ROWS_MAX_SETS];
+  const ddp_rows_range_t* ranges[DDP_ROWS_MAX_SETS];
+} ddp_rows_split_t;
+extern int ddp_rows_split;
+int ddp_conv_rows_split(const ddp_conv_shape_t* shape, const ddp_conv_task_t* tasks, int ntasks, const ddp_rows_split_t* splits, void* stream);
+int ddp_conv_rows_split_plan(const ddp_conv_shape_t* shape, const ddp_conv_task_t* tasks, int ntasks, const ddp_rows_split_t* splits, int32_t info[4]);
+
 typedef struct {
   const float* msg;
   const int32_t* rowptr;
```

Result: no change. 178.9, median of 2 (+0.3%).
